# bharath5673/StrongSORT-YOLO

Hardware: AMD Instinct MI355X
Metric: tracked frames/sec (whole node), 1280x720@30det (higher is better)
Workload: dtype f32 association / f64 Kalman+LSAP (f16 detector convs, fp32 ReID network on own v_mfma_f32 kernels)

## Files before the change

strongsort_yolo_amd/csrc/ss_front.hip:

```cpp
#include <hip/hip_fp16.h>
#include "ss_common.h"

__device__ inline void ss_axis(int d, float scale, int n_src, int& i0, int& i1, float& frac)
{
    float t = (float)d + 0.5f;
    float s = t * scale;
    float f = s - 0.5f;
    int i = (int)floorf(f);
    float fr = f - (float)i;
    if (i < 0) { i = 0; fr = 0.0f; }
    if (i >= n_src - 1) { i = n_src - 1; fr = 0.0f; i1 = i; } else i1 = i + 1;
    i0 = i; frac = fr;
}

__device__ inline float ss_bilerp_u8(float p00, float p01, float p10, float p11, float fx, float fy)
{
    float a = fmaf(fx, p01 - p00, p00);
    float b = fmaf(fx, p11 - p10, p10);
    float v = fmaf(fy, b - a, a);
    float q = floorf(v + 0.5f);
    return fminf(fmaxf(q, 0.0f), 255.0f);
}

template <typename T> __device__ inline T ss_cvt(float v);
template <> __device__ inline float ss_cvt<float>(float v) { return v; }
template <> __device__ inline __half ss_cvt<__half>(float v) { return __float2half(v); }
template <typename T> struct ss_is_u8 { static constexpr bool value = false; };
template <> struct ss_is_u8<uint8_t> { static constexpr bool value = true; };

template <typename T, int HWC>
__global__ __launch_bounds__(256) void k_letterbox(const uint8_t* __restrict__ src, long long src_batch_stride,
                                                   int H, int W, int stride, T* __restrict__ dst, int out_h,
                                                   int out_w, int new_h, int new_w, int pad_top, int pad_left,
                                                   float padv)
{
    const int x = blockIdx.x * blockDim.x + threadIdx.x;
    const int y = blockIdx.y;
    if (x >= out_w) return;
    const size_t plane = (size_t)out_h * out_w;
    src += (size_t)blockIdx.z * src_batch_stride;
    dst += (size_t)blockIdx.z * 3 * plane;
    const size_t o = HWC ? ((size_t)y * out_w + x) * 3 : (size_t)y * out_w + x;
    const size_t cs = HWC ? 1 : plane;
    const int ry = y - pad_top, rx = x - pad_left;
    if (ry < 0 || ry >= new_h || rx < 0 || rx >= new_w) {
        T p = ss_cvt<T>(padv);
        dst[o] = p; dst[cs + o] = p; dst[2 * cs + o] = p;
        return;
    }
    const float sx = (float)W / (float)new_w, sy = (float)H / (float)new_h;
    int y0, y1, x0, x1; float fy, fx;
    ss_axis(ry, sy, H, y0, y1, fy);
    ss_axis(rx, sx, W, x0, x1, fx);
    const uint8_t* r0 = src + (size_t)y0 * stride;
    const uint8_t* r1 = src + (size_t)y1 * stride;
#pragma unroll
    for (int c = 0; c < 3; ++c) {
        const int sc = 2 - c;
        float p00 = r0[x0 * 3 + sc], p01 = r0[x1 * 3 + sc], p10 = r1[x0 * 3 + sc], p11 = r1[x1 * 3 + sc];
        dst[c * cs + o] = ss_cvt<T>(ss_bilerp_u8(p00, p01, p10, p11, fx, fy) / 255.0f);
    }
}

void ss_launch_letterbox(const uint8_t* src, int batch, long long src_batch_stride, int h, int w, int stride, void* dst,
                         int flags, int out_h, int out_w, int new_h, int new_w, int pad_top, int pad_left,
                         int pad_value, hipStream_t st)
{
    if (batch <= 0) return;
    dim3 grid((out_w + 255) / 256, out_h, batch), block(256);
    float padv = (float)pad_value / 255.0f;
#define SS_LB(T, L) hipLaunchKernelGGL((k_letterbox<T, L>), grid, block, 0, st, src, src_batch_stride, h, w, stride, \
                                       (T*)dst, out_h, out_w, new_h, new_w, pad_top, pad_left, padv)
    switch (flags & 3) {
    case 0: SS_LB(float, 0); break;
    case 1: SS_LB(__half, 0); break;
    case 2: SS_LB(float, 1); break;
    default: SS_LB(__half, 1); break;
    }
#undef SS_LB
}

template <typename T, int HWC>
__global__ __launch_bounds__(128) void k_crop(const uint8_t* __restrict__ src, long long src_batch_stride, int H, int W,
                                              int stride, const float* __restrict__ dets, int det_stride,
                                              long long dets_batch_stride, int n, const int* __restrict__ d_count,
                                              T* __restrict__ dst)
{
    const int out_w = 128, out_h = 256;
    const int img = blockIdx.z / n, d = blockIdx.z - img * n;
    const int cnt = d_count ? d_count[img] : n;
    if (d >= cnt) return;
    src += (size_t)img * src_batch_stride;
    const int x = threadIdx.x, y = blockIdx.y;
    const float* b = dets + (size_t)img * dets_batch_stride + (size_t)d * det_stride;
    int x1 = (int)b[0], y1 = (int)b[1], x2 = (int)b[2], y2 = (int)b[3];
    if (x1 < 0) x1 = 0; if (y1 < 0) y1 = 0;
    if (x2 > W - 1) x2 = W - 1; if (y2 > H - 1) y2 = H - 1;
    if (x1 > W - 1) x1 = W - 1; if (y1 > H - 1) y1 = H - 1;
    int cw = x2 - x1, ch = y2 - y1;
    if (cw < 1) cw = 1; if (ch < 1) ch = 1;
    const float sx = (float)cw / (float)out_w, sy = (float)ch / (float)out_h;
    int yy0, yy1, xx0, xx1; float fy, fx;
    ss_axis(y, sy, ch, yy0, yy1, fy);
    ss_axis(x, sx, cw, xx0, xx1, fx);
    const uint8_t* r0 = src + (size_t)(y1 + yy0) * stride;
    const uint8_t* r1 = src + (size_t)(y1 + yy1) * stride;
    const float mean[3] = { 0.485f, 0.456f, 0.406f }, sd[3] = { 0.229f, 0.224f, 0.225f };
    const size_t plane = (size_t)out_h * out_w;
    T* o = dst + (size_t)blockIdx.z * 3 * plane + (HWC ? ((size_t)y * out_w + x) * 3 : (size_t)y * out_w + x);
    const size_t cs = HWC ? 1 : plane;
#pragma unroll
    for (int c = 0; c < 3; ++c) {
        const int sc = 2 - c;
        float p00 = r0[(x1 + xx0) * 3 + sc], p01 = r0[(x1 + xx1) * 3 + sc];
        float p10 = r1[(x1 + xx0) * 3 + sc], p11 = r1[(x1 + xx1) * 3 + sc];
        float q = ss_bilerp_u8(p00, p01, p10, p11, fx, fy) / 255.0f;
        o[c * cs] = ss_cvt<T>((q - mean[c]) / sd[c]);
    }
}

#define CROP_LDS_BYTES 30720
#define CROP_RPT 4

template <typename T>
__global__ __launch_bounds__(256) void k_crop_hwc8(const uint8_t* __restrict__ src, long long src_batch_stride, int H, int W,
                                                   int stride, const float* __restrict__ dets, int det_stride,
                                                   long long dets_batch_stride, int n, const int* __restrict__ d_count,
                                                   T* __restrict__ dst, const int* __restrict__ d_off)
{
    extern __shared__ __attribute__((aligned(16))) unsigned char crop_smem[];
    T* lut = reinterpret_cast<T*>(crop_smem);
    uint32_t* Ls = reinterpret_cast<uint32_t*>(crop_smem + 768 * sizeof(T));
    const int out_w = 128, out_h = 256;
    const int img = blockIdx.z / n, d = blockIdx.z - img * n;
    const int cnt = d_count ? d_count[img] : n;
    if (d >= cnt) return;
    src += (size_t)img * src_batch_stride;
    const int tid = threadIdx.x, yb = blockIdx.y * (16 * CROP_RPT), xg = (tid & 15) * 8;
    const float* b = dets + (size_t)img * dets_batch_stride + (size_t)d * det_stride;
    int x1 = (int)b[0], y1 = (int)b[1], x2 = (int)b[2], y2 = (int)b[3];
    if (x1 < 0) x1 = 0; if (y1 < 0) y1 = 0;
    if (x2 > W - 1) x2 = W - 1; if (y2 > H - 1) y2 = H - 1;
    if (x1 > W - 1) x1 = W - 1; if (y1 > H - 1) y1 = H - 1;
    int cw = x2 - x1, ch = y2 - y1;
    if (cw < 1) cw = 1; if (ch < 1) ch = 1;
    const float sx = (float)cw / (float)out_w, sy = (float)ch / (float)out_h;
    const float mean[3] = { 0.485f, 0.456f, 0.406f }, sd[3] = { 0.229f, 0.224f, 0.225f };
    for (int i = tid; i < 768; i += 256) {
        const int c = i >> 8;
        const float q = (float)(i & 255) / 255.0f;
        if constexpr (ss_is_u8<T>::value) lut[i] = (uint8_t)(i & 255);
        else lut[i] = ss_cvt<T>((q - mean[c]) / sd[c]);
    }
    int ra0, ra1, rb0, rb1; float fa, fb;
    ss_axis(yb, sy, ch, ra0, ra1, fa);
    ss_axis(yb + 16 * CROP_RPT - 1, sy, ch, rb0, rb1, fb);
    const int nrows = rb1 - ra0 + 1;
    const size_t rowb = (size_t)x1 * 3;
    const int mis = (int)(rowb & 3), ndw = (mis + cw * 3 + 3) >> 2, pitch = ndw + 1;
    const bool aligned = (stride & 3) == 0 && ((uintptr_t)src & 3) == 0;
    bool fit_sub = aligned;
#pragma unroll
    for (int rr = 0; rr < CROP_RPT; ++rr) {
        int a0, a1, b0, b1; float f0, f1;
        ss_axis(yb + 16 * rr, sy, ch, a0, a1, f0);
        ss_axis(yb + 16 * rr + 15, sy, ch, b0, b1, f1);
        fit_sub = fit_sub && (size_t)(b1 - a0 + 1) * pitch * 4 <= CROP_LDS_BYTES;
    }
    const int mode = (aligned && (size_t)nrows * pitch * 4 <= CROP_LDS_BYTES) ? 2 : fit_sub ? 1 : 0;
    const bool staged = mode != 0;
    const size_t end = (size_t)H * stride;
    auto stage = [&](const int r_first, const int nr) {
        const int tot = nr * ndw;
        for (int i0 = tid; i0 < tot; i0 += 256 * 8) {
            uint32_t v[8];
            int la[8];
#pragma unroll
            for (int u = 0; u < 8; ++u) {
                const int i = i0 + 256 * u;
                v[u] = 0; la[u] = -1;
                if (i < tot) {
                    const int rr = i / ndw, dw = i - rr * ndw;
                    const size_t off = (size_t)(y1 + r_first + rr) * stride + (rowb - mis) + (size_t)dw * 4;
                    la[u] = rr * pitch + dw;
                    if (off + 4 <= end) v[u] = *reinterpret_cast<const uint32_t*>(src + off);
                    else { for (int k = 0; k < 4 && off + k < end; ++k) v[u] |= (uint32_t)src[off + k] << (8 * k); }
                }
            }
#pragma unroll
            for (int u = 0; u < 8; ++u) if (la[u] >= 0) Ls[la[u]] = v[u];
        }
    };
    if (mode == 2) stage(ra0, nrows);
    __syncthreads();
    const size_t slot = d_off ? (size_t)d_off[img] + d : (size_t)blockIdx.z;
    int hob0[8], hob1[8];
    float hfx[8];
#pragma unroll
    for (int p = 0; p < 8; ++p) {
        int xx0, xx1;
        ss_axis(xg + p, sx, cw, xx0, xx1, hfx[p]);
        hob0[p] = mis + 3 * xx0; hob1[p] = mis + 3 * xx1;
    }
#pragma unroll 1
    for (int rr = 0; rr < CROP_RPT; ++rr) {
    const int y = yb + rr * 16 + (tid >> 4);
    int yy0, yy1; float fy;
    ss_axis(y, sy, ch, yy0, yy1, fy);
    __attribute__((aligned(16))) T o[24];
    if (staged) {
        int row0 = ra0;
        if (mode == 1) {
            int a1, b0, b1; float f0, f1;
            ss_axis(yb + 16 * rr, sy, ch, row0, a1, f0);
            ss_axis(yb + 16 * rr + 15, sy, ch, b0, b1, f1);
            if (rr) __syncthreads();
            stage(row0, b1 - row0 + 1);
            __syncthreads();
        }
        const uint32_t* l0 = Ls + (yy0 - row0) * pitch;
        const uint32_t* l1 = Ls + (yy1 - row0) * pitch;
        auto px = [&](const uint32_t* row, int ob) -> uint32_t {
            const int dw = ob >> 2;
            const uint64_t two = ((uint64_t)row[dw + 1] << 32) | row[dw];
            return (uint32_t)(two >> (8 * (ob & 3)));
        };
#pragma unroll
        for (int p = 0; p < 8; ++p) {
            const float fx = hfx[p];
            const uint32_t v00 = px(l0, hob0[p]), v01 = px(l0, hob1[p]), v10 = px(l1, hob0[p]), v11 = px(l1, hob1[p]);
#pragma unroll
            for (int c = 0; c < 3; ++c) {
                const int sh = 8 * (2 - c);
                const float p00 = (float)((v00 >> sh) & 255u), p01 = (float)((v01 >> sh) & 255u), p10 = (float)((v10 >> sh) & 255u),
                            p11 = (float)((v11 >> sh) & 255u);
                o[p * 3 + c] = lut[c * 256 + (int)ss_bilerp_u8(p00, p01, p10, p11, fx, fy)];
            }
        }
    } else {
        const uint8_t* r0 = src + (size_t)(y1 + yy0) * stride + rowb;
        const uint8_t* r1 = src + (size_t)(y1 + yy1) * stride + rowb;
        T* od = dst + (slot * out_h * out_w + (size_t)y * out_w + xg) * 3;
#pragma unroll 1
        for (int p = 0; p < 8; ++p) {
            int xx0, xx1; float fx;
            ss_axis(xg + p, sx, cw, xx0, xx1, fx);
#pragma unroll
            for (int c = 0; c < 3; ++c) {
                const int sc = 2 - c;
                const float p00 = r0[xx0 * 3 + sc], p01 = r0[xx1 * 3 + sc], p10 = r1[xx0 * 3 + sc], p11 = r1[xx1 * 3 + sc];
                od[p * 3 + c] = lut[c * 256 + (int)ss_bilerp_u8(p00, p01, p10, p11, fx, fy)];
            }
        }
        continue;
    }
    if constexpr (ss_is_u8<T>::value) {
        uint2* out = reinterpret_cast<uint2*>(dst + (slot * out_h * out_w + (size_t)y * out_w + xg) * 3);
        const uint2* ov = reinterpret_cast<const uint2*>(o);
#pragma unroll
        for (int v = 0; v < 3; ++v) out[v] = ov[v];
    } else {
        constexpr int NV = 24 * sizeof(T) / 16;
        uint4* out = reinterpret_cast<uint4*>(dst + (slot * out_h * out_w + (size_t)y * out_w + xg) * 3);
        const uint4* ov = reinterpret_cast<const uint4*>(o);
#pragma unroll
        for (int v = 0; v < NV; ++v) out[v] = ov[v];
    }
    }
}

__global__ __launch_bounds__(1024) void k_crop_offsets(const int* __restrict__ counts, int batch, int n, int* __restrict__ off)
{
    __shared__ int wtot[16];
    const int tid = threadIdx.x, lane = tid & 63, wv = tid >> 6, per = (batch + 1023) / 1024, i0 = tid * per;
    int sum = 0;
    for (int i = i0; i < i0 + per && i < batch; ++i) sum += min(counts[i], n);
    int inc = sum;
#pragma unroll
    for (int o = 1; o < 64; o <<= 1) { const int t = __shfl_up(inc, o); if (lane >= o) inc += t; }
    if (lane == 63) wtot[wv] = inc;
    __syncthreads();
    int base = 0, total = 0;
#pragma unroll
    for (int i = 0; i < 16; ++i) { const int c = wtot[i]; if (i < wv) base += c; total += c; }
    int a = base + inc - sum;
    if (tid == 0) off[batch] = total;
    for (int i = i0; i < i0 + per && i < batch; ++i) { off[i] = a; a += min(counts[i], n); }
}

template <typename T>
__global__ __launch_bounds__(128) void k_unpack_feats(const T* __restrict__ emb, const int* __restrict__ off, const int* __restrict__ counts,
                                                     int n, float* __restrict__ feats, long long feats_img_stride)
{
    const int img = blockIdx.y, d = blockIdx.x;
    if (d >= min(counts[img], n)) return;
    const T* src = emb + ((size_t)off[img] + d) * 512;
    float* dst = feats + (size_t)img * feats_img_stride + (size_t)d * 512;
    for (int k = threadIdx.x; k < 512; k += 128) dst[k] = (float)src[k];
}

__global__ __launch_bounds__(256) void k_pack_results(const int* __restrict__ n_dets, const float* __restrict__ dets, int det_ld, int det_cap,
                                                      const int* __restrict__ n_out, const float* __restrict__ out, int out_ld, int out_cap,
                                                      float* __restrict__ dst)
{
    const int n = min(max(*n_dets, 0), det_cap), m = (n_out && out) ? min(max(*n_out, 0), out_cap) : 0;
    if (threadIdx.x == 0) { reinterpret_cast<int*>(dst)[0] = n; reinterpret_cast<int*>(dst)[1] = m; }
    float* d0 = dst + 2;
    for (int i = threadIdx.x; i < n * det_ld; i += 256) d0[i] = dets[i];
    float* d1 = dst + 2 + (size_t)det_cap * det_ld;
    for (int i = threadIdx.x; i < m * out_ld; i += 256) d1[i] = out[i];
}

void ss_launch_pack_results(const int* n_dets, const float* dets, int det_ld, int det_cap, const int* n_out, const float* out, int out_ld,
                            int out_cap, float* dst, hipStream_t st)
{ hipLaunchKernelGGL(k_pack_results, dim3(1), dim3(256), 0, st, n_dets, dets, det_ld, det_cap, n_out, out, out_ld, out_cap, dst); }

void ss_launch_crop_offsets(const int* counts, int batch, int n, int* off, hipStream_t st)
{ hipLaunchKernelGGL(k_crop_offsets, dim3(1), dim3(1024), 0, st, counts, batch, n, off); }

void ss_launch_unpack_feats(const void* emb, int half, const int* off, const int* counts, int batch, int n, float* feats,
                            long long feats_img_stride, hipStream_t st)
{
    if (batch <= 0 || n <= 0) return;
    if (half) hipLaunchKernelGGL(k_unpack_feats<__half>, dim3(n, batch), dim3(128), 0, st, (const __half*)emb, off, counts, n, feats, feats_img_stride);
    else hipLaunchKernelGGL(k_unpack_feats<float>, dim3(n, batch), dim3(128), 0, st, (const float*)emb, off, counts, n, feats, feats_img_stride);
}

void ss_launch_crop(const uint8_t* frame, int batch, long long frame_batch_stride, int h, int w, int stride,
                    const float* dets, int det_stride, long long dets_batch_stride, int n, const int* d_count,
                    void* out, int flags, hipStream_t st, const int* d_off)
{
    if (n <= 0 || batch <= 0) return;
    if (flags & 2) {
        dim3 grid(1, 16 / CROP_RPT, n * batch), block(256);
        if (flags & 4) { hipLaunchKernelGGL(k_crop_hwc8<uint8_t>, grid, block, 768 + CROP_LDS_BYTES + 8, st, frame, frame_batch_stride, h, w, stride, dets, det_stride, dets_batch_stride, n, d_count, (uint8_t*)out, d_off); return; }
        if (flags & 1) hipLaunchKernelGGL(k_crop_hwc8<__half>, grid, block, 768 * sizeof(__half) + CROP_LDS_BYTES + 8, st, frame, frame_batch_stride, h, w, stride, dets, det_stride, dets_batch_stride, n, d_count, (__half*)out, d_off);
        else           hipLaunchKernelGGL(k_crop_hwc8<float>, grid, block, 768 * sizeof(float) + CROP_LDS_BYTES + 8, st, frame, frame_batch_stride, h, w, stride, dets, det_stride, dets_batch_stride, n, d_count, (float*)out, d_off);
        return;
    }
    dim3 grid(1, 256, n * batch), block(128);
#define SS_CR(T, L) hipLaunchKernelGGL((k_crop<T, L>), grid, block, 0, st, frame, frame_batch_stride, h, w, stride, dets, \
                                       det_stride, dets_batch_stride, n, d_count, (T*)out)
    if (flags & 1) SS_CR(__half, 0); else SS_CR(float, 0);
#undef SS_CR
}

#define NMS_MAX_ANCHORS 32768
#define NMS_MAX_CAND 8192
#define NMS_WORDS (NMS_MAX_CAND / 64)

struct NmsWs {
    unsigned long long* keys;
    int* cand_cls;
    float* box;
    float* area;
    unsigned long long* mask;
    int* counters;
};

size_t ss_nms_workspace_bytes()
{
    return (size_t)NMS_MAX_ANCHORS * 8 + (size_t)NMS_MAX_ANCHORS * 4 + (size_t)NMS_MAX_CAND * 16 +
           (size_t)NMS_MAX_CAND * 4 + (size_t)NMS_MAX_CAND * NMS_WORDS * 8 + 64;
}

__host__ __device__ inline NmsWs carve_nms(void* ws)
{
    NmsWs w; char* p = (char*)ws;
    w.keys = (unsigned long long*)p; p += (size_t)NMS_MAX_ANCHORS * 8;
    w.mask = (unsigned long long*)p; p += (size_t)NMS_MAX_CAND * NMS_WORDS * 8;
    w.box = (float*)p; p += (size_t)NMS_MAX_CAND * 16;
    w.area = (float*)p; p += (size_t)NMS_MAX_CAND * 4;
    w.cand_cls = (int*)p; p += (size_t)NMS_MAX_ANCHORS * 4;
    w.counters = (int*)p;
    return w;
}

struct NmsBatch {
    const float* pred; long long pred_stride;
    char* ws; long long ws_stride;
};
__device__ inline NmsWs nms_unit(const NmsBatch& nb, int img) { return carve_nms(nb.ws + (size_t)img * nb.ws_stride); }

__global__ __launch_bounds__(512) void k_nms_filter(NmsBatch nb, int N, int nc, float conf, unsigned long long cm0,
                                                    unsigned long long cm1)
{
    const float* __restrict__ pred = nb.pred + (size_t)blockIdx.y * nb.pred_stride;
    const NmsWs w = nms_unit(nb, blockIdx.y);
    __shared__ float sbest[8][64];
    __shared__ int scls[8][64];
    const int g = threadIdx.x >> 6, l = threadIdx.x & 63;
    const int a = blockIdx.x * 64 + l;
    float best = -INFINITY; int bc = 0x7fffffff;
    if (a < N)
        for (int k0 = g; k0 < nc; k0 += 80) {
            float s[10];
#pragma unroll
            for (int j = 0; j < 10; ++j) s[j] = pred[(size_t)(4 + min(k0 + 8 * j, nc - 1)) * N + a];
#pragma unroll
            for (int j = 0; j < 10; ++j) {
                const int k = k0 + 8 * j;
                if (k < nc && s[j] > best) { best = s[j]; bc = k; }
            }
        }
    sbest[g][l] = best; scls[g][l] = bc;
    __syncthreads();
    if (g != 0 || a >= N) return;
#pragma unroll
    for (int q = 1; q < 8; ++q) {
        float s = sbest[q][l]; int c = scls[q][l];
        if (s > best || (s == best && c < bc)) { best = s; bc = c; }
    }
    const bool allowed = bc < 64 ? (cm0 >> bc) & 1ull : bc < 128 ? (cm1 >> (bc - 64)) & 1ull : true;
    if (best > conf && allowed) {
        int slot = atomicAdd(&w.counters[0], 1);
        w.keys[slot] = ((unsigned long long)(~__float_as_uint(best)) << 32) | (unsigned)a;
        w.cand_cls[a] = bc;
    }
}

__global__ __launch_bounds__(1024) void k_nms_sort(NmsBatch nb, int N, int agnostic, float max_wh)
{
    const float* __restrict__ pred = nb.pred + (size_t)blockIdx.x * nb.pred_stride;
    const NmsWs w = nms_unit(nb, blockIdx.x);
    extern __shared__ __attribute__((aligned(16))) char smem[];
    unsigned long long* k = (unsigned long long*)smem;
    int n = w.counters[0];
    __syncthreads();
    if (n > NMS_MAX_CAND) {
        if (threadIdx.x == 0) { w.counters[1] = SS_ERR_CAPACITY; w.counters[0] = 0; }
        n = 0;
    }
    int np = 1; while (np < n) np <<= 1;
    for (int i = threadIdx.x; i < np; i += 1024) k[i] = i < n ? w.keys[i] : ~0ull;
    __syncthreads();
    for (int size = 2; size <= np; size <<= 1)
        for (int strd = size >> 1; strd > 0; strd >>= 1) {
            for (int i = threadIdx.x; i < np / 2; i += 1024) {
                int lo = 2 * i - (i & (strd - 1)), hi = lo + strd;
                bool up = (lo & size) == 0;
                unsigned long long a = k[lo], b = k[hi];
                if ((a > b) == up) { k[lo] = b; k[hi] = a; }
            }
            __syncthreads();
        }
    for (int i = threadIdx.x; i < n; i += 1024) {
        unsigned long long key = k[i];
        w.keys[i] = key;
        const int a = (int)(key & 0xffffffffu);
        float cx = pred[a], cy = pred[(size_t)N + a], bw = pred[(size_t)2 * N + a], bh = pred[(size_t)3 * N + a];
        float hw = bw / 2.0f, hh = bh / 2.0f;
        float off = agnostic ? 0.0f : (float)w.cand_cls[a] * max_wh;
        float x1 = (cx - hw) + off, y1 = (cy - hh) + off, x2 = (cx + hw) + off, y2 = (cy + hh) + off;
        w.box[i * 4 + 0] = x1; w.box[i * 4 + 1] = y1; w.box[i * 4 + 2] = x2; w.box[i * 4 + 3] = y2;
        w.area[i] = (x2 - x1) * (y2 - y1);
    }
}

#define NMS_MASK_WG 256
__global__ __launch_bounds__(64) void k_nms_mask(NmsBatch nb, float iou_thres)
{
    const NmsWs w = nms_unit(nb, blockIdx.y);
    __shared__ float sb[64 * 4];
    __shared__ float sa[64];
    const int n = min(w.counters[0], NMS_MAX_CAND);
    const int nblk = (n + 63) / 64;
    const int npair = nblk * (nblk + 1) / 2;
    const int t = threadIdx.x;
    for (int pr = blockIdx.x; pr < npair; pr += gridDim.x) {
        int ib = 0, rem = pr;
        while (rem >= nblk - ib) { rem -= nblk - ib; ++ib; }
        const int jb = ib + rem;
        const int j = jb * 64 + t;
        __syncthreads();
        if (j < n) { sb[t * 4] = w.box[j * 4]; sb[t * 4 + 1] = w.box[j * 4 + 1]; sb[t * 4 + 2] = w.box[j * 4 + 2]; sb[t * 4 + 3] = w.box[j * 4 + 3]; sa[t] = w.area[j]; }
        __syncthreads();
        const int i = ib * 64 + t;
        if (i >= n) continue;
        const float x1 = w.box[i * 4], y1 = w.box[i * 4 + 1], x2 = w.box[i * 4 + 2], y2 = w.box[i * 4 + 3], ai = w.area[i];
        unsigned long long bits = 0;
        const int jn = min(64, n - jb * 64);
        for (int q = 0; q < jn; ++q) {
            if (jb * 64 + q <= i) continue;
            float xx1 = fmaxf(x1, sb[q * 4]), yy1 = fmaxf(y1, sb[q * 4 + 1]);
            float xx2 = fminf(x2, sb[q * 4 + 2]), yy2 = fminf(y2, sb[q * 4 + 3]);
            float iw = fmaxf(0.0f, xx2 - xx1), ih = fmaxf(0.0f, yy2 - yy1);
            float inter = iw * ih;
            float iou = inter / (ai + sa[q] - inter);
            if (iou > iou_thres) bits |= 1ull << q;
        }
        w.mask[(size_t)i * NMS_WORDS + jb] = bits;
    }
}

__global__ __launch_bounds__(64) void k_nms_scan(NmsBatch nb, int N, int nc, int n_extra, int max_det, float gain,
                                                 float pad_x, float pad_y, float w0, float h0,
                                                 const float* __restrict__ geom, float* __restrict__ rows,
                                                 int row_stride, long long rows_batch_stride, int* __restrict__ keep,
                                                 long long keep_batch_stride, int* __restrict__ count)
{
    const int img = blockIdx.x;
    const float* __restrict__ pred = nb.pred + (size_t)img * nb.pred_stride;
    const NmsWs w = nms_unit(nb, img);
    rows += (size_t)img * rows_batch_stride; keep += (size_t)img * keep_batch_stride; count += img;
    if (geom) { const float* g = geom + img * 5; gain = g[0]; pad_x = g[1]; pad_y = g[2]; w0 = g[3]; h0 = g[4]; }
    __shared__ int kept_sorted[1024];
    const int n = min(w.counters[0], NMS_MAX_CAND);
    const int l = threadIdx.x;
    const int nw = (n + 63) / 64;
    unsigned long long rem0 = 0, rem1 = 0;
    int kept = 0;
    const int cap = min(max_det, 1024);
    for (int ib = 0; ib < nw && kept < cap; ++ib) {
        unsigned long long rw = __shfl((ib < 64) ? rem0 : rem1, ib & 63);
        const int i0 = ib * 64;
        const int cnt = min(64, n - i0);
        unsigned long long diag = (l < cnt) ? w.mask[(size_t)(i0 + l) * NMS_WORDS + ib] : 0ull;
        unsigned long long keptbits = 0;
        for (int q = 0; q < cnt && kept < cap; ++q) {
            if (!((rw >> q) & 1ull)) {
                keptbits |= 1ull << q;
                if (l == 0) kept_sorted[kept] = i0 + q;
                ++kept;
                rw |= __shfl(diag, q);
            }
        }
        unsigned long long kb = keptbits;
        while (kb) {
            int q[4];
#pragma unroll
            for (int u = 0; u < 4; ++u) { q[u] = kb ? __builtin_ctzll(kb) : -1; if (kb) kb &= kb - 1; }
            unsigned long long a0[4], a1[4];
#pragma unroll
            for (int u = 0; u < 4; ++u) {
                a0[u] = a1[u] = 0ull;
                if (q[u] >= 0) {
                    const unsigned long long* mr = w.mask + (size_t)(i0 + q[u]) * NMS_WORDS;
                    if (l > ib && l < nw) a0[u] = mr[l];
                    if (l + 64 > ib && l + 64 < nw) a1[u] = mr[l + 64];
                }
            }
            rem0 |= (a0[0] | a0[1]) | (a0[2] | a0[3]);
            rem1 |= (a1[0] | a1[1]) | (a1[2] | a1[3]);
        }
    }
    __syncthreads();
    if (l == 0) { *count = kept; w.counters[0] = 0; }
    for (int kk = l; kk < kept; kk += 64) {
        const int i = kept_sorted[kk];
        const unsigned long long key = w.keys[i];
        const int a = (int)(key & 0xffffffffu);
        const float score = __uint_as_float(~(unsigned)(key >> 32));
        float cx = pred[a], cy = pred[(size_t)N + a], bw = pred[(size_t)2 * N + a], bh = pred[(size_t)3 * N + a];
        float hw = bw / 2.0f, hh = bh / 2.0f;
        float x1 = ((cx - hw) - pad_x) / gain, y1 = ((cy - hh) - pad_y) / gain;
        float x2 = ((cx + hw) - pad_x) / gain, y2 = ((cy + hh) - pad_y) / gain;
        float* r = rows + (size_t)kk * row_stride;
        r[0] = fminf(fmaxf(x1, 0.0f), w0); r[1] = fminf(fmaxf(y1, 0.0f), h0);
        r[2] = fminf(fmaxf(x2, 0.0f), w0); r[3] = fminf(fmaxf(y2, 0.0f), h0);
        r[4] = score; r[5] = (float)w.cand_cls[a];
        for (int e = 0; e < n_extra; ++e) r[6 + e] = pred[(size_t)(4 + nc + e) * N + a];
        keep[kk] = a;
    }
}

__global__ __launch_bounds__(1024) void k_nms_rest(NmsBatch nb, int N, int nc, int n_extra, int agnostic, float max_wh, float iou_thres,
                                                   int max_det, float gain, float pad_x, float pad_y, float w0, float h0,
                                                   const float* __restrict__ geom, float* __restrict__ rows, int row_stride,
                                                   long long rows_batch_stride, int* __restrict__ keep, long long keep_batch_stride,
                                                   int* __restrict__ count)
{
    const int img = blockIdx.x;
    const float* __restrict__ pred = nb.pred + (size_t)img * nb.pred_stride;
    const NmsWs w = nms_unit(nb, img);
    rows += (size_t)img * rows_batch_stride; keep += (size_t)img * keep_batch_stride; count += img;
    if (geom) { const float* g = geom + img * 5; gain = g[0]; pad_x = g[1]; pad_y = g[2]; w0 = g[3]; h0 = g[4]; }
    extern __shared__ __attribute__((aligned(16))) char smem[];
    unsigned long long* k = (unsigned long long*)smem;
    float* sbw = (float*)(smem + (size_t)NMS_MAX_CAND * 8);
    float* saw = sbw + 16 * 64 * 4;
    int* kept_sorted = (int*)(saw + 16 * 64);
    __shared__ int s_kept;
    const int tid = threadIdx.x, l = tid & 63, wv = tid >> 6;
    int n = w.counters[0];
    __syncthreads();
    if (n > NMS_MAX_CAND) {
        if (tid == 0) { w.counters[1] = SS_ERR_CAPACITY; w.counters[0] = 0; }
        n = 0;
    }
    if (n <= 64) {
        if (wv == 0) {
            unsigned long long key = l < n ? w.keys[l] : ~0ull;
            auto shfl64 = [](unsigned long long v, int src) {
                const unsigned lo = (unsigned)__shfl((int)(unsigned)v, src), hi = (unsigned)__shfl((int)(unsigned)(v >> 32), src);
                return ((unsigned long long)hi << 32) | lo;
            };
#pragma unroll
            for (int size = 2; size <= 64; size <<= 1)
#pragma unroll
                for (int strd = size >> 1; strd > 0; strd >>= 1) {
                    const unsigned long long other = shfl64(key, l ^ strd);
                    const bool lower = (l & strd) == 0, up = (l & size) == 0;
                    const bool take_min = lower == up;
                    key = take_min ? (key < other ? key : other) : (key > other ? key : other);
                }
            float x1 = 0.f, y1 = 0.f, x2 = 0.f, y2 = 0.f, ai = 0.f;
            if (l < n) {
                w.keys[l] = key;
                const int a = (int)(key & 0xffffffffu);
                float cx = pred[a], cy = pred[(size_t)N + a], bw = pred[(size_t)2 * N + a], bh = pred[(size_t)3 * N + a];
                float hw = bw / 2.0f, hh = bh / 2.0f;
                float off = agnostic ? 0.0f : (float)w.cand_cls[a] * max_wh;
                x1 = (cx - hw) + off; y1 = (cy - hh) + off; x2 = (cx + hw) + off; y2 = (cy + hh) + off;
                ai = (x2 - x1) * (y2 - y1);
                sbw[l * 4] = x1; sbw[l * 4 + 1] = y1; sbw[l * 4 + 2] = x2; sbw[l * 4 + 3] = y2; saw[l] = ai;
            }
            SS_WAVE_SYNC();
            unsigned long long bits = 0;
            if (l < n) {
                for (int q = 0; q < n; ++q) {
                    if (q <= l) continue;
                    float xx1 = fmaxf(x1, sbw[q * 4]), yy1 = fmaxf(y1, sbw[q * 4 + 1]);
                    float xx2 = fminf(x2, sbw[q * 4 + 2]), yy2 = fminf(y2, sbw[q * 4 + 3]);
                    float iw = fmaxf(0.0f, xx2 - xx1), ih = fmaxf(0.0f, yy2 - yy1);
                    float inter = iw * ih;
                    float iou = inter / (ai + saw[q] - inter);
                    if (iou > iou_thres) bits |= 1ull << q;
                }
            }
            unsigned long long rw = 0;
            int kept = 0;
            const int cap = min(max_det, 1024);
            for (int q = 0; q < n && kept < cap; ++q) {
                if (!((rw >> q) & 1ull)) {
                    if (l == 0) kept_sorted[kept] = q;
                    ++kept;
                    rw |= shfl64(bits, q);
// ... 160 lines not shown
```

strongsort_yolo_amd/csrc/ss_ops.hip:

```cpp
#include <hip/hip_fp16.h>
#include <hip/hip_runtime.h>
#include <stdint.h>
#include <stdlib.h>
#include <string>
#include "../../include/strongsort_hip.h"

struct NvEntry { void* stream; const int* n; int batch; };
static thread_local NvEntry g_nv[8] = {};
static inline const int* nv_for(void* stream, long long batch)
{
    for (const NvEntry& e : g_nv) if (e.n && e.stream == stream && e.batch == batch) return e.n;
    return nullptr;
}
static inline int nv_batch(void* stream)
{
    for (const NvEntry& e : g_nv) if (e.n && e.stream == stream) return e.batch;
    return 0;
}

static int g_opt_pw_epilogue = 1, g_opt_pw_splitk = 1, g_opt_osnet_chains = 1;

typedef _Float16 h8 __attribute__((ext_vector_type(8)));
typedef _Float16 h4 __attribute__((ext_vector_type(4)));
typedef float f4 __attribute__((ext_vector_type(4)));

__device__ inline float act_apply(float v, int act)
{
    if (act == 1) return v > 0.f ? v : 0.f;
    if (act == 2) return v * __builtin_amdgcn_rcpf(1.0f + __expf(-v));
    if (act == 3) return __builtin_amdgcn_rcpf(1.0f + __expf(-v));
    return v;
}

__global__ __launch_bounds__(256) void k_bias_act8(__half* __restrict__ x, const __half* __restrict__ bias,
                                                  const __half* __restrict__ res, size_t n_vec, int C8, int act)
{
    for (size_t i = blockIdx.x * (size_t)blockDim.x + threadIdx.x; i < n_vec; i += (size_t)gridDim.x * blockDim.x) {
        h8 v = reinterpret_cast<h8*>(x)[i];
        h8 b = reinterpret_cast<const h8*>(bias)[i % C8];
        h8 r;
        if (res) r = reinterpret_cast<const h8*>(res)[i];
#pragma unroll
        for (int k = 0; k < 8; ++k) {
            float f = (float)v[k] + (float)b[k];
            if (res) f += (float)r[k];
            v[k] = (_Float16)act_apply(f, act);
        }
        reinterpret_cast<h8*>(x)[i] = v;
    }
}

__global__ __launch_bounds__(256) void k_bias_act1(__half* __restrict__ x, const __half* __restrict__ bias,
                                                  const __half* __restrict__ res, size_t n, int C, int act)
{
    for (size_t i = blockIdx.x * (size_t)blockDim.x + threadIdx.x; i < n; i += (size_t)gridDim.x * blockDim.x) {
        float f = __half2float(x[i]) + __half2float(bias[i % C]);
        if (res) f += __half2float(res[i]);
        x[i] = __float2half(act_apply(f, act));
    }
}

__device__ __forceinline__ float ss_mix_lo(unsigned a, unsigned b, float c)
{ float d; asm("v_fma_mix_f32 %0, %1, %2, %3 op_sel:[0,0,0] op_sel_hi:[1,1,0]" : "=v"(d) : "v"(a), "v"(b), "v"(c)); return d; }
__device__ __forceinline__ float ss_mix_hi(unsigned a, unsigned b, float c)
{ float d; asm("v_fma_mix_f32 %0, %1, %2, %3 op_sel:[1,1,0] op_sel_hi:[1,1,0]" : "=v"(d) : "v"(a), "v"(b), "v"(c)); return d; }
__device__ __forceinline__ void ss_dw_tap8(const h8& v, const h8& w, float (&acc)[8])
{
    const uint4 vu = __builtin_bit_cast(uint4, v), wu = __builtin_bit_cast(uint4, w);
    acc[0] = ss_mix_lo(vu.x, wu.x, acc[0]); acc[1] = ss_mix_hi(vu.x, wu.x, acc[1]);
    acc[2] = ss_mix_lo(vu.y, wu.y, acc[2]); acc[3] = ss_mix_hi(vu.y, wu.y, acc[3]);
    acc[4] = ss_mix_lo(vu.z, wu.z, acc[4]); acc[5] = ss_mix_hi(vu.z, wu.z, acc[5]);
    acc[6] = ss_mix_lo(vu.w, wu.w, acc[6]); acc[7] = ss_mix_hi(vu.w, wu.w, acc[7]);
}

__global__ __launch_bounds__(256) void k_dw3x3(const __half* __restrict__ x, const __half* __restrict__ w9,
                                              const __half* __restrict__ bias, __half* __restrict__ y, int N, int H,
                                              int W, int C8, int act)
{
    const size_t total = (size_t)N * H * W * C8;
    for (size_t i = blockIdx.x * (size_t)blockDim.x + threadIdx.x; i < total; i += (size_t)gridDim.x * blockDim.x) {
        const int c8 = (int)(i % C8);
        const size_t p = i / C8;
        const int w = (int)(p % W), h = (int)((p / W) % H);
        const size_t nb = (p / ((size_t)W * H)) * H;
        float acc[8];
        {
            h8 b = reinterpret_cast<const h8*>(bias)[c8];
#pragma unroll
            for (int k = 0; k < 8; ++k) acc[k] = (float)b[k];
        }
#pragma unroll
        for (int dy = -1; dy <= 1; ++dy) {
            const int hh = h + dy;
            if (hh < 0 || hh >= H) continue;
#pragma unroll
            for (int dx = -1; dx <= 1; ++dx) {
                const int ww = w + dx;
                if (ww < 0 || ww >= W) continue;
                h8 v = reinterpret_cast<const h8*>(x)[((nb + hh) * W + ww) * C8 + c8];
                h8 k9 = reinterpret_cast<const h8*>(w9)[((dy + 1) * 3 + dx + 1) * C8 + c8];
                ss_dw_tap8(v, k9, acc);
            }
        }
        h8 o;
#pragma unroll
        for (int k = 0; k < 8; ++k) o[k] = (_Float16)act_apply(acc[k], act);
        reinterpret_cast<h8*>(y)[i] = o;
    }
}

__global__ __launch_bounds__(256) void k_bias_act_place(const __half* __restrict__ x, const __half* __restrict__ bias,
                                                       const __half* __restrict__ res, size_t n_vec, int C8, int act,
                                                       int res_after, __half* __restrict__ out, int out_ld8,
                                                       __half* __restrict__ out2, int c0_8, int cn_8)
{
    for (size_t i = blockIdx.x * (size_t)blockDim.x + threadIdx.x; i < n_vec; i += (size_t)gridDim.x * blockDim.x) {
        const size_t pix = i / C8;
        const int c8 = (int)(i - pix * C8);
        h8 v = reinterpret_cast<const h8*>(x)[i];
        const h8 b = reinterpret_cast<const h8*>(bias)[c8];
        h8 r;
        if (res) r = reinterpret_cast<const h8*>(res)[i];
#pragma unroll
        for (int k = 0; k < 8; ++k) {
            float f = (float)v[k] + (float)b[k];
            if (res && !res_after) f += (float)r[k];
            f = act_apply(f, act);
            if (res && res_after) f = (float)(_Float16)f + (float)r[k];
            v[k] = (_Float16)f;
        }
        reinterpret_cast<h8*>(out)[pix * out_ld8 + c8] = v;
        if (out2 && c8 >= c0_8 && c8 < c0_8 + cn_8) reinterpret_cast<h8*>(out2)[pix * cn_8 + (c8 - c0_8)] = v;
    }
}

struct V8Levels {
    const __half* box[3]; const __half* cls[3];
    const __half* box_bias[3]; const __half* cls_bias[3];
    int H[3], W[3], stride[3];
    const __half* ext[3];
    int n_ext, ext_ld, ext_mode;
    int cls_ld;
};

__global__ __launch_bounds__(128) void k_v8_decode(V8Levels L, int B, int nc, int A, float* __restrict__ pred)
{
    const int a = blockIdx.x * blockDim.x + threadIdx.x, b = blockIdx.y;
    if (a >= A) return;
    int l = 0, a0 = 0;
    while (l < 2 && a >= a0 + L.H[l] * L.W[l]) { a0 += L.H[l] * L.W[l]; ++l; }
    const int p = a - a0, hw = L.H[l] * L.W[l];
    const int py = p / L.W[l], px = p - py * L.W[l];
    const h8* bx = reinterpret_cast<const h8*>(L.box[l] + ((size_t)b * hw + p) * 64);
    const h8* bb = reinterpret_cast<const h8*>(L.box_bias[l]);
    float d[4];
#pragma unroll
    for (int s = 0; s < 4; ++s) {
        float v[16], m = -INFINITY;
#pragma unroll
        for (int h = 0; h < 2; ++h) {
            const h8 t = bx[s * 2 + h], tb = bb[s * 2 + h];
#pragma unroll
            for (int k = 0; k < 8; ++k) { v[h * 8 + k] = (float)t[k] + (float)tb[k]; m = fmaxf(m, v[h * 8 + k]); }
        }
        float se = 0.f, sw = 0.f;
#pragma unroll
        for (int k = 0; k < 16; ++k) { const float e = __expf(v[k] - m); se += e; sw += e * (float)k; }
        d[s] = sw / se;
    }
    const float ax = (float)px + 0.5f, ay = (float)py + 0.5f, st = (float)L.stride[l];
    const float x1 = ax - d[0], y1 = ay - d[1], x2 = ax + d[2], y2 = ay + d[3];
    float* o = pred + (size_t)b * (4 + nc + L.n_ext) * A + a;
    o[0] = (x1 + x2) * 0.5f * st; o[(size_t)A] = (y1 + y2) * 0.5f * st;
    o[(size_t)2 * A] = (x2 - x1) * st; o[(size_t)3 * A] = (y2 - y1) * st;
    if (L.n_ext) {
        const __half* e = L.ext[l] + ((size_t)b * hw + p) * L.ext_ld;
        float* oe = o + (size_t)(4 + nc) * A;
        for (int k = 0, j = 0; k < L.n_ext; ++k, j = j == 2 ? 0 : j + 1) {
            const float v = __half2float(e[k]);
            oe[(size_t)k * A] = L.ext_mode == 0 ? v : j == 0 ? (v * 2.0f + (float)px) * st : j == 1 ? (v * 2.0f + (float)py) * st : 1.0f / (1.0f + __expf(-v));
        }
    }
    const __half* cl = L.cls[l] + ((size_t)b * hw + p) * L.cls_ld;
    const __half* cb = L.cls_bias[l];
    if (nc % 8 == 0) {
        for (int k8 = 0; k8 < nc / 8; ++k8) {
            const h8 t = reinterpret_cast<const h8*>(cl)[k8], tb = reinterpret_cast<const h8*>(cb)[k8];
#pragma unroll
            for (int k = 0; k < 8; ++k) o[(size_t)(4 + k8 * 8 + k) * A] = 1.0f / (1.0f + __expf(-((float)t[k] + (float)tb[k])));
        }
        return;
    }
    for (int k = 0; k < nc; ++k) {
        const float z = __half2float(cl[k]) + __half2float(cb[k]);
        o[(size_t)(4 + k) * A] = 1.0f / (1.0f + __expf(-z));
    }
}

struct ConvGeom { int H, W, Cin, OH, OW, stride; };

struct PwArgs {
    const __half* x; const __half* w; const __half* bias; const __half* res;
    int M, K, N, act, res_after;
    __half* out; int out_ld; __half* out2; int c0, cn;
    ConvGeom g;
    const int* n_img; int img_px;
};

template <int BN, int PT, bool VEC_EPI>
constexpr int pw_lds_halfs() { return BN * 72 + (VEC_EPI ? 4 * PT * 16 * (BN + 8) : 0); }

template <int BN, int PT, bool CONV3, bool VEC_EPI>
__device__ __forceinline__ void pw_body(const PwArgs& A, const int bx, const int by, _Float16* __restrict__ pw_lds)
{
    const __half* __restrict__ x = A.x; const __half* __restrict__ w = A.w; const __half* __restrict__ bias = A.bias;
    const __half* __restrict__ res = A.res; __half* __restrict__ out = A.out; __half* __restrict__ out2 = A.out2;
    const int K = A.K, N = A.N, act = A.act, res_after = A.res_after, out_ld = A.out_ld, c0 = A.c0, cn = A.cn;
    int M = A.M;
    if (A.n_img) { const long long mv = (long long)(*A.n_img) * A.img_px; if (mv < M) M = (int)mv; }
    const ConvGeom g = A.g;
    constexpr int MT = BN / 16, KC = 64, PITCH = KC + 8, BM = 64 * PT;
    if ((long long)bx * BM >= M) return;
    _Float16* __restrict__ Ws = pw_lds;
    const int tid = threadIdx.x, lane = tid & 63, wave = tid >> 6, q = lane >> 4, n = lane & 15;
    const int n0 = by * BN;
    const size_t px0 = (size_t)bx * BM + wave * (16 * PT);
    f4 acc[MT][PT];
#pragma unroll
    for (int mt = 0; mt < MT; ++mt)
#pragma unroll
        for (int pt = 0; pt < PT; ++pt) acc[mt][pt] = f4{ 0.f, 0.f, 0.f, 0.f };
    const h8 z8 = { 0, 0, 0, 0, 0, 0, 0, 0 };
    size_t ibase[PT];
    int iy0[PT], ix0[PT];
    if (CONV3) {
#pragma unroll
        for (int pt = 0; pt < PT; ++pt) {
            const size_t px = px0 + pt * 16 + n;
            const int ohw = g.OH * g.OW;
            const int bimg = (int)(px / ohw), rem = (int)(px - (size_t)bimg * ohw), oy = rem / g.OW, ox = rem - oy * g.OW;
            ibase[pt] = (size_t)bimg * g.H * g.W;
            iy0[pt] = oy * g.stride - 1; ix0[pt] = ox * g.stride - 1;
        }
    }

    constexpr int WV = (BN * (KC / 8) + 255) / 256;
    auto load_w = [&](int kc, h8 (&wr)[WV]) {
#pragma unroll
        for (int j = 0; j < WV; ++j) {
            const int i = tid + j * 256, r = i / (KC / 8), c8 = i - r * (KC / 8);
            const int oc = n0 + r, k = kc + c8 * 8;
            wr[j] = (i < BN * (KC / 8) && oc < N && k < K) ? *reinterpret_cast<const h8*>(w + (size_t)oc * K + k) : z8;
        }
    };
    auto load_b = [&](int kc, h8 (&b)[KC / 32][PT]) {
#pragma unroll
        for (int ks = 0; ks < KC / 32; ++ks)
#pragma unroll
            for (int pt = 0; pt < PT; ++pt) {
                const size_t px = px0 + pt * 16 + n;
                const int k = kc + ks * 32 + 8 * q;
                if (!CONV3) {
                    b[ks][pt] = (px < (size_t)M && k < K) ? *reinterpret_cast<const h8*>(x + px * K + k) : z8;
                } else {
                    const int tap = k / g.Cin, c = k - tap * g.Cin, dy = tap / 3, dx = tap - dy * 3;
                    const int iy = iy0[pt] + dy, ix = ix0[pt] + dx;
                    const bool ok = px < (size_t)M && k < K && iy >= 0 && iy < g.H && ix >= 0 && ix < g.W;
                    b[ks][pt] = ok ? *reinterpret_cast<const h8*>(x + (ibase[pt] + (size_t)iy * g.W + ix) * g.Cin + c) : z8;
                }
            }
    };
    h8 wr[WV], wn[WV], b[KC / 32][PT], bn[KC / 32][PT];
    load_w(0, wr);
    load_b(0, b);
    for (int kc = 0; kc < K; kc += KC) {
        __syncthreads();
#pragma unroll
        for (int j = 0; j < WV; ++j) {
            const int i = tid + j * 256, r = i / (KC / 8), c8 = i - r * (KC / 8);
            if (i < BN * (KC / 8)) *reinterpret_cast<h8*>(Ws + r * PITCH + c8 * 8) = wr[j];
        }
        if (kc + KC < K) { load_w(kc + KC, wn); load_b(kc + KC, bn); }
        __syncthreads();
#pragma unroll
        for (int ks = 0; ks < KC / 32; ++ks) {
            if (kc + ks * 32 >= K) break;
#pragma unroll
            for (int mt = 0; mt < MT; ++mt) {
                const h8 a = *reinterpret_cast<const h8*>(Ws + (mt * 16 + n) * PITCH + ks * 32 + 8 * q);
                const h4 a0 = { a[0], a[1], a[2], a[3] }, a1 = { a[4], a[5], a[6], a[7] };
#pragma unroll
                for (int pt = 0; pt < PT; ++pt) {
                    const h8 bv = b[ks][pt];
                    if (CONV3) {
                        acc[mt][pt] = __builtin_amdgcn_mfma_f32_16x16x32_f16(a, bv, acc[mt][pt], 0, 0, 0);
                    } else {
                        const h4 b0 = { bv[0], bv[1], bv[2], bv[3] }, b1 = { bv[4], bv[5], bv[6], bv[7] };
                        acc[mt][pt] = __builtin_amdgcn_mfma_f32_16x16x16f16(a0, b0, acc[mt][pt], 0, 0, 0);
                        acc[mt][pt] = __builtin_amdgcn_mfma_f32_16x16x16f16(a1, b1, acc[mt][pt], 0, 0, 0);
                    }
                }
            }
        }
        if (kc + KC < K) {
#pragma unroll
            for (int j = 0; j < WV; ++j) wr[j] = wn[j];
#pragma unroll
            for (int ks = 0; ks < KC / 32; ++ks)
#pragma unroll
                for (int pt = 0; pt < PT; ++pt) b[ks][pt] = bn[ks][pt];
        }
    }

    if (VEC_EPI) {
        constexpr int EP = BN + 8;
        _Float16* tile = pw_lds + BN * PITCH + wave * (PT * 16 * EP);
#pragma unroll
        for (int pt = 0; pt < PT; ++pt)
#pragma unroll
            for (int mt = 0; mt < MT; ++mt) {
                const h4 o = { (_Float16)acc[mt][pt][0], (_Float16)acc[mt][pt][1], (_Float16)acc[mt][pt][2], (_Float16)acc[mt][pt][3] };
                *reinterpret_cast<h4*>(tile + (pt * 16 + n) * EP + mt * 16 + 4 * q) = o;
            }
        __builtin_amdgcn_wave_barrier();
        constexpr int CG = BN / 8;
#pragma unroll
        for (int it = 0; it < (PT * 16 * CG + 63) / 64; ++it) {
            const int i = it * 64 + lane, row = i / CG, cg = i - row * CG;
            const size_t px = px0 + row;
            const int oc = n0 + cg * 8;
            if (i >= PT * 16 * CG || px >= (size_t)M || oc >= N) continue;
            const h8 v = *reinterpret_cast<const h8*>(tile + row * EP + cg * 8);
            const h8 bb = *reinterpret_cast<const h8*>(bias + oc);
            h8 r = z8;
            if (res) r = *reinterpret_cast<const h8*>(res + px * N + oc);
            h8 o;
#pragma unroll
            for (int j = 0; j < 8; ++j) {
                float f = (float)v[j] + (float)bb[j];
                if (res && !res_after) f += (float)r[j];
                f = act_apply(f, act);
                if (res && res_after) f = (float)(_Float16)f + (float)r[j];
                o[j] = (_Float16)f;
            }
            *reinterpret_cast<h8*>(out + px * out_ld + oc) = o;
            if (out2 && oc >= c0 && oc < c0 + cn) *reinterpret_cast<h8*>(out2 + px * cn + (oc - c0)) = o;
        }
        return;
    }
#pragma unroll
    for (int pt = 0; pt < PT; ++pt) {
        const size_t px = px0 + pt * 16 + n;
        if (px >= (size_t)M) continue;
#pragma unroll
        for (int mt = 0; mt < MT; ++mt) {
            const int oc0 = n0 + mt * 16 + 4 * q;
            if (oc0 >= N) continue;
            const h4 bb = *reinterpret_cast<const h4*>(bias + oc0);
            h4 r = { 0, 0, 0, 0 };
            if (res) r = *reinterpret_cast<const h4*>(res + px * N + oc0);
            h4 o;
#pragma unroll
            for (int j = 0; j < 4; ++j) {
                float f = (float)(_Float16)acc[mt][pt][j] + (float)bb[j];
                if (res && !res_after) f += (float)r[j];
                f = act_apply(f, act);
                if (res && res_after) f = (float)(_Float16)f + (float)r[j];
                o[j] = (_Float16)f;
            }
            *reinterpret_cast<h4*>(out + px * out_ld + oc0) = o;
            if (out2 && oc0 >= c0 && oc0 < c0 + cn) *reinterpret_cast<h4*>(out2 + px * cn + (oc0 - c0)) = o;
        }
    }
}

#ifndef SS_TAIL_BUMP
#define SS_TAIL_BUMP 1
#endif
#ifndef SS_PW_BUMP
#define SS_PW_BUMP 1
#endif
template <int BN, int PT, bool CONV3> constexpr int pw_waves() { return !SS_PW_BUMP ? 1 : BN * PT <= 32 ? 8 : (BN == 32 && PT == 2 && CONV3) ? 5 : BN * PT <= 80 ? 6 : BN * PT <= 128 ? 4 : BN * PT <= 160 ? 3 : 2; }
template <int BN, int PT, bool CONV3, bool VEC_EPI>
__global__ __launch_bounds__(256) __attribute__((amdgpu_waves_per_eu(pw_waves<BN, PT, CONV3>()))) void k_pw(PwArgs A)
{
    __shared__ __attribute__((aligned(16))) _Float16 pw_lds[pw_lds_halfs<BN, PT, VEC_EPI>()];
    pw_body<BN, PT, CONV3, VEC_EPI>(A, blockIdx.x, blockIdx.y, pw_lds);
}

template <int BN, bool CONV3>
__device__ __forceinline__ void pw_splitk_body(const PwArgs& A, const int bx, const int by)
{
    const __half* __restrict__ x = A.x; const __half* __restrict__ w = A.w; const __half* __restrict__ bias = A.bias;
    const __half* __restrict__ res = A.res; __half* __restrict__ out = A.out; __half* __restrict__ out2 = A.out2;
    const int K = A.K, N = A.N, act = A.act, res_after = A.res_after, out_ld = A.out_ld, c0 = A.c0, cn = A.cn;
    int M = A.M;
    if (A.n_img) { const long long mv = (long long)(*A.n_img) * A.img_px; if (mv < M) M = (int)mv; }
    const ConvGeom g = A.g;
    constexpr int MT = BN / 16, KC = 64, RP = 17;
    __shared__ float Red[4 * BN * RP];
    const int tid = threadIdx.x, lane = tid & 63, wave = tid >> 6, q = lane >> 4, n = lane & 15;
    const int n0 = by * BN;
    const size_t px = (size_t)bx * 16 + n;
    const h8 z8 = { 0, 0, 0, 0, 0, 0, 0, 0 };
    size_t ibase = 0;
    int iy0 = 0, ix0 = 0;
    if (CONV3) {
        const int ohw = g.OH * g.OW;
        const int bimg = (int)(px / ohw), rem = (int)(px - (size_t)bimg * ohw), oy = rem / g.OW, ox = rem - oy * g.OW;
        ibase = (size_t)bimg * g.H * g.W;
        iy0 = oy * g.stride - 1; ix0 = ox * g.stride - 1;
    }
    auto load_a = [&](int kc, h8 (&a)[MT][2]) {
#pragma unroll
        for (int mt = 0; mt < MT; ++mt)
#pragma unroll
            for (int ks = 0; ks < 2; ++ks) {
                const int oc = n0 + mt * 16 + n, k = kc + ks * 32 + 8 * q;
                a[mt][ks] = (oc < N && k < K) ? *reinterpret_cast<const h8*>(w + (size_t)oc * K + k) : z8;
            }
    };
    auto load_b = [&](int kc, h8 (&b)[2]) {
#pragma unroll
        for (int ks = 0; ks < 2; ++ks) {
            const int k = kc + ks * 32 + 8 * q;
            if (!CONV3) {
                b[ks] = (px < (size_t)M && k < K) ? *reinterpret_cast<const h8*>(x + px * K + k) : z8;
            } else {
                const int tap = k / g.Cin, c = k - tap * g.Cin, dy = tap / 3, dx = tap - dy * 3;
                const int iy = iy0 + dy, ix = ix0 + dx;
                const bool ok = px < (size_t)M && k < K && iy >= 0 && iy < g.H && ix >= 0 && ix < g.W;
                b[ks] = ok ? *reinterpret_cast<const h8*>(x + (ibase + (size_t)iy * g.W + ix) * g.Cin + c) : z8;
            }
        }
    };
    f4 acc[MT];
#pragma unroll
    for (int mt = 0; mt < MT; ++mt) acc[mt] = f4{ 0.f, 0.f, 0.f, 0.f };
    h8 a[MT][2], b[2], an[MT][2], bn[2];
    int kc = wave * KC;
    if (kc < K) { load_a(kc, a); load_b(kc, b); }
    for (; kc < K; kc += 4 * KC) {
        const bool more = kc + 4 * KC < K;
        if (more) { load_a(kc + 4 * KC, an); load_b(kc + 4 * KC, bn); }
#pragma unroll
        for (int ks = 0; ks < 2; ++ks) {
            if (kc + ks * 32 >= K) break;
#pragma unroll
            for (int mt = 0; mt < MT; ++mt) acc[mt] = __builtin_amdgcn_mfma_f32_16x16x32_f16(a[mt][ks], b[ks], acc[mt], 0, 0, 0);
        }
        if (more) {
#pragma unroll
            for (int mt = 0; mt < MT; ++mt) { a[mt][0] = an[mt][0]; a[mt][1] = an[mt][1]; }
            b[0] = bn[0]; b[1] = bn[1];
        }
    }
#pragma unroll
    for (int mt = 0; mt < MT; ++mt)
#pragma unroll
        for (int j = 0; j < 4; ++j) Red[(wave * BN + mt * 16 + 4 * q + j) * RP + n] = acc[mt][j];
    __syncthreads();
    constexpr int CG = BN / 8;
    if (tid < 16 * CG) {
        const int row = tid / CG, cg = tid - row * CG;
        const size_t p = (size_t)bx * 16 + row;
        const int oc = n0 + cg * 8;
        if (p < (size_t)M && oc < N) {
            const h8 bb = *reinterpret_cast<const h8*>(bias + oc);
            h8 r = z8;
            if (res) r = *reinterpret_cast<const h8*>(res + p * N + oc);
            h8 o;
#pragma unroll
            for (int j = 0; j < 8; ++j) {
                const int ch = cg * 8 + j;
                const float sum = ((Red[(0 * BN + ch) * RP + row] + Red[(1 * BN + ch) * RP + row]) + Red[(2 * BN + ch) * RP + row]) +
                                  Red[(3 * BN + ch) * RP + row];
                float f = (float)(_Float16)sum + (float)bb[j];
                if (res && !res_after) f += (float)r[j];
                f = act_apply(f, act);
                if (res && res_after) f = (float)(_Float16)f + (float)r[j];
                o[j] = (_Float16)f;
            }
            *reinterpret_cast<h8*>(out + p * out_ld + oc) = o;
            if (out2 && oc >= c0 && oc < c0 + cn) *reinterpret_cast<h8*>(out2 + p * cn + (oc - c0)) = o;
        }
    }
}

template <int BN, bool CONV3>
__global__ __launch_bounds__(256) void k_pw_splitk(PwArgs A) { pw_splitk_body<BN, CONV3>(A, blockIdx.x, blockIdx.y); }

#define PW_GROUP_MAX 12
struct PwGroup { PwArgs p[PW_GROUP_MAX]; int start[PW_GROUP_MAX + 1]; int form[PW_GROUP_MAX]; int n; };

#ifndef SS_GRP_WAVES
#define SS_GRP_WAVES 6
#endif
template <int BN, bool CONV3, bool SPLITK>
__global__ __launch_bounds__(256)
__attribute__((amdgpu_waves_per_eu(SPLITK || !SS_GRP_WAVES ? 1 : SS_GRP_WAVES)))
void k_pw_group(PwGroup G)
{
    __shared__ __attribute__((aligned(16))) _Float16 pw_lds[pw_lds_halfs<BN, 1, true>()];
    int bx = blockIdx.x, p = 0;
    for (int i = 1; i < G.n; ++i) if (bx >= G.start[i]) p = i;
    bx -= G.start[p];
    const int form = G.form[p];
    if constexpr (SPLITK) { if (form == 1) { pw_splitk_body<BN, CONV3>(G.p[p], bx, 0); return; } }
    if (BN == 80 && G.p[p].N <= 64) pw_body<64, 1, CONV3, true>(G.p[p], bx, 0, pw_lds);
    else pw_body<BN, 1, CONV3, true>(G.p[p], bx, 0, pw_lds);
}

struct BnArgs {
    const __half* x; const __half* w1; const __half* b1; const __half* w2; const __half* b2;
    __half* out; int out_ld; __half* out2;
    int B, H, W, add, TW, TH, tiles_x, tiles_y;
};

template <int CI, int CO, int PT>
__device__ __forceinline__ void bn_conv(const _Float16* __restrict__ In, const int (&pbase)[PT], const int* __restrict__ tapoff,
                                        const __half* __restrict__ w, _Float16* __restrict__ Ws, f4 (&acc)[CO / 16][PT], const int tid)
{
    constexpr int C = CI;
    constexpr int MT = CO / 16, WP = 72, K = 9 * CI, WV = (CO * 8 + 255) / 256;
    const int lane = tid & 63, q = lane >> 4, n = lane & 15;
    const h8 z8 = { 0, 0, 0, 0, 0, 0, 0, 0 };
    auto load_w = [&](int k0, h8 (&wr)[WV]) {
#pragma unroll
        for (int j = 0; j < WV; ++j) {
            const int i = tid + j * 256, r = i >> 3, c8 = i & 7, kk = k0 + c8 * 8;
            wr[j] = (i < CO * 8 && kk < K) ? *reinterpret_cast<const h8*>(w + (size_t)r * K + kk) : z8;
        }
    };
    h8 wr[WV], wn[WV];
    load_w(0, wr);
    int buf = 0;
    for (int k0 = 0; k0 < K; k0 += 64, buf ^= 1) {
        _Float16* wb = Ws + buf * (CO * WP);
#pragma unroll
        for (int j = 0; j < WV; ++j) {
            const int i = tid + j * 256, r = i >> 3, c8 = i & 7;
            if (i < CO * 8) *reinterpret_cast<h8*>(wb + r * WP + c8 * 8) = wr[j];
        }
        if (k0 + 64 < K) load_w(k0 + 64, wn);
        __syncthreads();
        h8 b[2][PT], a[2][MT];
#pragma unroll
        for (int ks = 0; ks < 2; ++ks) {
            const int kk = k0 + ks * 32 + 8 * q, tap = kk / C, c = kk % C;
            const bool kv = kk < K;
            const int boff = kv ? tapoff[tap] + c : 0;
#pragma unroll
            for (int pt = 0; pt < PT; ++pt) {
                b[ks][pt] = *reinterpret_cast<const h8*>(In + pbase[pt] + boff);
                if (!kv) b[ks][pt] = z8;
            }
#pragma unroll
            for (int mt = 0; mt < MT; ++mt) a[ks][mt] = *reinterpret_cast<const h8*>(wb + (mt * 16 + n) * WP + ks * 32 + 8 * q);
        }
#pragma unroll
        for (int ks = 0; ks < 2; ++ks) {
            if (k0 + ks * 32 >= K) break;
#pragma unroll
            for (int mt = 0; mt < MT; ++mt)
#pragma unroll
                for (int pt = 0; pt < PT; ++pt)
                    acc[mt][pt] = __builtin_amdgcn_mfma_f32_16x16x32_f16(a[ks][mt], b[ks][pt], acc[mt][pt], 0, 0, 0);
        }
        if (k0 + 64 < K) {
#pragma unroll
            for (int j = 0; j < WV; ++j) wr[j] = wn[j];
        }
    }
}

template <int C, int PT1, int PT2>
__global__ __launch_bounds__(256) __attribute__((amdgpu_waves_per_eu(!SS_TAIL_BUMP ? 1 : C == 16 ? 6 : 1))) void k_bneck(BnArgs A)
{
    extern __shared__ __attribute__((aligned(16))) char bn_smem[];
    constexpr int MT = C / 16, P = C + 8, WP = 72;
    const int tid = threadIdx.x, lane = tid & 63, wave = tid >> 6, q = lane >> 4, n = lane & 15;
    const int TW = A.TW, TH = A.TH, XW = TW + 4, XH = TH + 4, RW = TW + 2, RH = TH + 2;
    _Float16* Xs = reinterpret_cast<_Float16*>(bn_smem);
    _Float16* Ts = Xs + XH * XW * P;
    _Float16* Ws = Ts + ((RH * RW * P + 7) & ~7);
    int* tap1 = reinterpret_cast<int*>(Ws + 2 * C * WP);
    int* tap2 = tap1 + 16;
    const int tpi = A.tiles_x * A.tiles_y;
    const int img = blockIdx.x / tpi, trm = blockIdx.x - img * tpi, tyi = trm / A.tiles_x, txi = trm - tyi * A.tiles_x;
    const int oy0 = tyi * TH, ox0 = txi * TW, H = A.H, W = A.W;
    const h8 z8 = { 0, 0, 0, 0, 0, 0, 0, 0 };
    if (tid < 9) { const int ky = tid / 3, kx = tid - ky * 3; tap1[tid] = (ky * XW + kx) * P; tap2[tid] = (ky * RW + kx) * P; }
    const __half* xi = A.x + (size_t)img * H * W * C;
    constexpr int VPC = C / 8;
    const int rowv = XW * VPC;
    for (int r = wave; r < XH; r += 4) {
        const int iy = oy0 - 2 + r;
        const bool rok = iy >= 0 && iy < H;
        const __half* src = xi + (size_t)(rok ? iy : 0) * W * C;
        _Float16* dst = Xs + r * XW * P;
        for (int i0 = lane; i0 < rowv; i0 += 512) {
            h8 tmp[8];
#pragma unroll
            for (int u = 0; u < 8; ++u) {
                const int i = i0 + 64 * u, c = i / VPC, v = i % VPC, ix = ox0 - 2 + c;
                const bool ok = rok && i < rowv && ix >= 0 && ix < W;
                tmp[u] = ok ? *reinterpret_cast<const h8*>(src + (size_t)ix * C + v * 8) : z8;
            }
#pragma unroll
            for (int u = 0; u < 8; ++u) {
                const int i = i0 + 64 * u, c = i / VPC, v = i % VPC;
                if (i < rowv) *reinterpret_cast<h8*>(dst + c * P + v * 8) = tmp[u];
            }
        }
    }
    {
        int pb[PT1], tpix[PT1];
        bool inimg[PT1];
#pragma unroll
        for (int pt = 0; pt < PT1; ++pt) {
            const int p = (wave * PT1 + pt) * 16 + n;
            int ry = p / RW, rx = p - ry * RW;
            const bool ok = p < RH * RW;
            if (!ok) { ry = 0; rx = 0; }
            const int iy = oy0 - 1 + ry, ix = ox0 - 1 + rx;
            inimg[pt] = ok && iy >= 0 && iy < H && ix >= 0 && ix < W;
            tpix[pt] = ok ? p : -1;
            pb[pt] = (ry * XW + rx) * P;
        }
        f4 acc[MT][PT1];
#pragma unroll
        for (int mt = 0; mt < MT; ++mt)
#pragma unroll
            for (int pt = 0; pt < PT1; ++pt) acc[mt][pt] = f4{ 0.f, 0.f, 0.f, 0.f };
        bn_conv<C, C, PT1>(Xs, pb, tap1, A.w1, Ws, acc, tid);
#pragma unroll
        for (int mt = 0; mt < MT; ++mt) {
            const h4 bb = *reinterpret_cast<const h4*>(A.b1 + mt * 16 + 4 * q);
#pragma unroll
            for (int pt = 0; pt < PT1; ++pt) {
                if (tpix[pt] < 0) continue;
                h4 o;
#pragma unroll
                for (int j = 0; j < 4; ++j) {
                    float f = act_apply((float)(_Float16)acc[mt][pt][j] + (float)bb[j], 2);
                    asm volatile("" : "+v"(f));
                    o[j] = inimg[pt] ? (_Float16)f : (_Float16)0.f;
                }
                *reinterpret_cast<h4*>(Ts + tpix[pt] * P + mt * 16 + 4 * q) = o;
            }
        }
    }
    __syncthreads();
    {
        int pb[PT2], opix[PT2], xoff[PT2];
#pragma unroll
        for (int pt = 0; pt < PT2; ++pt) {
            const int p = (wave * PT2 + pt) * 16 + n;
            int ty = p / TW, tx = p - ty * TW;
            const bool ok = p < TH * TW && oy0 + ty < H && ox0 + tx < W;
            if (!ok) { ty = 0; tx = 0; }
            pb[pt] = (ty * RW + tx) * P;
            xoff[pt] = ((ty + 2) * XW + tx + 2) * P;
            opix[pt] = ok ? (img * H + oy0 + ty) * W + ox0 + tx : -1;
        }
        f4 acc[MT][PT2];
#pragma unroll
        for (int mt = 0; mt < MT; ++mt)
#pragma unroll
            for (int pt = 0; pt < PT2; ++pt) acc[mt][pt] = f4{ 0.f, 0.f, 0.f, 0.f };
        bn_conv<C, C, PT2>(Ts, pb, tap2, A.w2, Ws, acc, tid);
#pragma unroll
        for (int mt = 0; mt < MT; ++mt) {
            const h4 bb = *reinterpret_cast<const h4*>(A.b2 + mt * 16 + 4 * q);
#pragma unroll
            for (int pt = 0; pt < PT2; ++pt) {
                if (opix[pt] < 0) continue;
                const h4 xr = *reinterpret_cast<const h4*>(Xs + xoff[pt] + mt * 16 + 4 * q);
                h4 o;
#pragma unroll
                for (int j = 0; j < 4; ++j) {
                    float f = act_apply((float)(_Float16)acc[mt][pt][j] + (float)bb[j], 2);
                    asm volatile("" : "+v"(f));
                    if (A.add) f = (float)(_Float16)f + (float)xr[j];
                    o[j] = (_Float16)f;
                }
                *reinterpret_cast<h4*>(A.out + (size_t)opix[pt] * A.out_ld + mt * 16 + 4 * q) = o;
                if (A.out2) *reinterpret_cast<h4*>(A.out2 + (size_t)opix[pt] * C + mt * 16 + 4 * q) = o;
            }
        }
    }
}

struct HeadArgs {
    const __half* x;
    const __half* w1[2]; const __half* b1[2]; const __half* w2[2]; const __half* b2[2]; const __half* w3[2]; const __half* b3[2];
    __half* out[2]; int nout[2];
    int B, H, W, TW, TH, tiles_x, tiles_y;
};

template <int CI, int CM, int PT1, int PT2>
__device__ __forceinline__ void head_body(const HeadArgs& A, const int br, char* smem)
{
    constexpr int MT = CM / 16, PX = CI + 8, PM = CM + 8, WP = 72, KB3 = (CM + 31) / 32;
    const int tid = threadIdx.x, lane = tid & 63, wave = tid >> 6, q = lane >> 4, n = lane & 15;
    const int TW = A.TW, TH = A.TH, XW = TW + 4, XH = TH + 4, RW = TW + 2, RH = TH + 2;
    _Float16* Xs = reinterpret_cast<_Float16*>(smem);
    _Float16* Ts = Xs + ((XH * XW * PX + 7) & ~7);
    _Float16* Ws = Ts + ((RH * RW * PM + 7) & ~7);
    int* tap1 = reinterpret_cast<int*>(Ws + 2 * 80 * WP);
    int* tap2 = tap1 + 16;
    _Float16* Us = Xs;
    const int tpi = A.tiles_x * A.tiles_y;
    const int img = blockIdx.x / tpi, trm = blockIdx.x - img * tpi, tyi = trm / A.tiles_x, txi = trm - tyi * A.tiles_x;
    const int oy0 = tyi * TH, ox0 = txi * TW, H = A.H, W = A.W;
    const h8 z8 = { 0, 0, 0, 0, 0, 0, 0, 0 };
    if (tid < 9) { const int ky = tid / 3, kx = tid - ky * 3; tap1[tid] = (ky * XW + kx) * PX; tap2[tid] = (ky * RW + kx) * PM; }
    const __half* xi = A.x + (size_t)img * H * W * CI;
    constexpr int VPC = CI / 8;
    const int rowv = XW * VPC;
    for (int r = wave; r < XH; r += 4) {
        const int iy = oy0 - 2 + r;
        const bool rok = iy >= 0 && iy < H;
        const __half* src = xi + (size_t)(rok ? iy : 0) * W * CI;
        _Float16* dst = Xs + r * XW * PX;
        for (int i0 = lane; i0 < rowv; i0 += 512) {
            h8 tmp[8];
#pragma unroll
            for (int u = 0; u < 8; ++u) {
                const int i = i0 + 64 * u, c = i / VPC, v = i % VPC, ix = ox0 - 2 + c;
                const bool ok = rok && i < rowv && ix >= 0 && ix < W;
                tmp[u] = ok ? *reinterpret_cast<const h8*>(src + (size_t)ix * CI + v * 8) : z8;
            }
#pragma unroll
            for (int u = 0; u < 8; ++u) {
                const int i = i0 + 64 * u, c = i / VPC, v = i % VPC;
                if (i < rowv) *reinterpret_cast<h8*>(dst + c * PX + v * 8) = tmp[u];
            }
        }
    }
    {
        int pb[PT1], tpix[PT1];
        bool inimg[PT1];
#pragma unroll
        for (int pt = 0; pt < PT1; ++pt) {
            const int p = (wave * PT1 + pt) * 16 + n;
            int ry = p / RW, rx = p - ry * RW;
            const bool ok = p < RH * RW;
            if (!ok) { ry = 0; rx = 0; }
            const int iy = oy0 - 1 + ry, ix = ox0 - 1 + rx;
            inimg[pt] = ok && iy >= 0 && iy < H && ix >= 0 && ix < W;
            tpix[pt] = ok ? p : -1;
            pb[pt] = (ry * XW + rx) * PX;
        }
        f4 acc[MT][PT1];
#pragma unroll
        for (int mt = 0; mt < MT; ++mt)
#pragma unroll
            for (int pt = 0; pt < PT1; ++pt) acc[mt][pt] = f4{ 0.f, 0.f, 0.f, 0.f };
        bn_conv<CI, CM, PT1>(Xs, pb, tap1, A.w1[br], Ws, acc, tid);
#pragma unroll
        for (int mt = 0; mt < MT; ++mt) {
            const h4 bb = *reinterpret_cast<const h4*>(A.b1[br] + mt * 16 + 4 * q);
#pragma unroll
            for (int pt = 0; pt < PT1; ++pt) {
                if (tpix[pt] < 0) continue;
                h4 o;
#pragma unroll
                for (int j = 0; j < 4; ++j) {
                    float f = act_apply((float)(_Float16)acc[mt][pt][j] + (float)bb[j], 2);
                    asm volatile("" : "+v"(f));
                    o[j] = inimg[pt] ? (_Float16)f : (_Float16)0.f;
                }
                *reinterpret_cast<h4*>(Ts + tpix[pt] * PM + mt * 16 + 4 * q) = o;
            }
        }
    }
    __syncthreads();
    int opix[PT2];
    {
        int pb[PT2];
#pragma unroll
        for (int pt = 0; pt < PT2; ++pt) {
            const int p = (wave * PT2 + pt) * 16 + n;
            int ty = p / TW, tx = p - ty * TW;
            const bool ok = p < TH * TW && oy0 + ty < H && ox0 + tx < W;
            if (!ok) { ty = 0; tx = 0; }
            pb[pt] = (ty * RW + tx) * PM;
            opix[pt] = ok ? (img * H + oy0 + ty) * W + ox0 + tx : -1;
        }
        f4 acc[MT][PT2];
#pragma unroll
        for (int mt = 0; mt < MT; ++mt)
#pragma unroll
            for (int pt = 0; pt < PT2; ++pt) acc[mt][pt] = f4{ 0.f, 0.f, 0.f, 0.f };
        bn_conv<CM, CM, PT2>(Ts, pb, tap2, A.w2[br], Ws, acc, tid);
        _Float16* ut = Us + wave * (PT2 * 16 * PM);
#pragma unroll
        for (int mt = 0; mt < MT; ++mt) {
            const h4 bb = *reinterpret_cast<const h4*>(A.b2[br] + mt * 16 + 4 * q);
#pragma unroll
            for (int pt = 0; pt < PT2; ++pt) {
                h4 o;
#pragma unroll
                for (int j = 0; j < 4; ++j) {
                    float f = act_apply((float)(_Float16)acc[mt][pt][j] + (float)bb[j], 2);
                    asm volatile("" : "+v"(f));
                    o[j] = (_Float16)f;
                }
                *reinterpret_cast<h4*>(ut + (pt * 16 + n) * PM + mt * 16 + 4 * q) = o;
            }
        }
    }
    __syncthreads();
    const int nout = A.nout[br];
    {
        const __half* w3 = A.w3[br];
        for (int i = tid; i < CM * (CM / 8); i += 256) {
            const int r = i / (CM / 8), c8 = i - r * (CM / 8);
            *reinterpret_cast<h8*>(Ws + r * PM + c8 * 8) = r < nout ? *reinterpret_cast<const h8*>(w3 + (size_t)r * CM + c8 * 8) : z8;
        }
    }
    __syncthreads();
    {
        const _Float16* ut = Us + wave * (PT2 * 16 * PM);
        f4 acc[MT][PT2];
#pragma unroll
        for (int mt = 0; mt < MT; ++mt)
#pragma unroll
            for (int pt = 0; pt < PT2; ++pt) acc[mt][pt] = f4{ 0.f, 0.f, 0.f, 0.f };
#pragma unroll
        for (int kb = 0; kb < KB3; ++kb) {
            const int k = kb * 32 + 8 * q;
            const bool kv = k < CM;
            h8 b[PT2];
#pragma unroll
            for (int pt = 0; pt < PT2; ++pt) b[pt] = kv ? *reinterpret_cast<const h8*>(ut + (pt * 16 + n) * PM + k) : z8;
#pragma unroll
            for (int mt = 0; mt < MT; ++mt) {
                const h8 a = kv ? *reinterpret_cast<const h8*>(Ws + (mt * 16 + n) * PM + k) : z8;
                const h4 a0 = { a[0], a[1], a[2], a[3] }, a1 = { a[4], a[5], a[6], a[7] };
#pragma unroll
                for (int pt = 0; pt < PT2; ++pt) {
                    const h4 b0 = { b[pt][0], b[pt][1], b[pt][2], b[pt][3] }, b1 = { b[pt][4], b[pt][5], b[pt][6], b[pt][7] };
                    acc[mt][pt] = __builtin_amdgcn_mfma_f32_16x16x16f16(a0, b0, acc[mt][pt], 0, 0, 0);
                    acc[mt][pt] = __builtin_amdgcn_mfma_f32_16x16x16f16(a1, b1, acc[mt][pt], 0, 0, 0);
                }
            }
        }
        __half* out = A.out[br];
#pragma unroll
        for (int mt = 0; mt < MT; ++mt) {
            const int oc0 = mt * 16 + 4 * q;
            if (oc0 >= nout) continue;
            const h4 bb = *reinterpret_cast<const h4*>(A.b3[br] + oc0);
#pragma unroll
            for (int pt = 0; pt < PT2; ++pt) {
                if (opix[pt] < 0) continue;
                h4 o;
#pragma unroll
                for (int j = 0; j < 4; ++j) o[j] = (_Float16)((float)(_Float16)acc[mt][pt][j] + (float)bb[j]);
                *reinterpret_cast<h4*>(out + (size_t)opix[pt] * nout + oc0) = o;
            }
        }
    }
}

template <int CI, int PT1, int PT2>
__global__ __launch_bounds__(256) void k_head(HeadArgs A)
{
    extern __shared__ __attribute__((aligned(16))) char hd_smem[];
    if (blockIdx.y == 0) head_body<CI, 64, PT1, PT2>(A, 0, hd_smem);
    else head_body<CI, 80, PT1, PT2>(A, 1, hd_smem);
}

#define STEM_W 128
#define STEM_M 16
#define STEM_PITCH 416
#define STEM_IN_ROWS 23
#define STEM_CR 9
#define STEM_CW 65
#define STEM_CP 18
typedef _Float16 h4a4 __attribute__((ext_vector_type(4), aligned(4)));
typedef _Float16 h8a4 __attribute__((ext_vector_type(8), aligned(4)));

__global__ __launch_bounds__(256) void k_osnet_stem(const __half* __restrict__ x, const __half* __restrict__ wp ,
                                                   const __half* __restrict__ bias, __half* __restrict__ y, int H, int tiles,
                                                   const int* __restrict__ nvalid, const __half* __restrict__ w1c,
                                                   const __half* __restrict__ b1c, __half* __restrict__ y1)
{
    if (nvalid && (int)(blockIdx.x / tiles) >= *nvalid) return;
    __shared__ __attribute__((aligned(16))) _Float16 In[STEM_IN_ROWS * STEM_PITCH];
    __shared__ __attribute__((aligned(16))) _Float16 Cv[STEM_CR * STEM_CW * STEM_CP];
    const int tid = threadIdx.x, lane = tid & 63, r = tid >> 6, q = lane >> 4, n = lane & 15;
    const int img = blockIdx.x / tiles, j0 = (blockIdx.x - img * tiles) * 4;
    const int OHc = H / 2, OHp = OHc / 2;
    const int in_r0 = 4 * j0 - 5, cv_r0 = 2 * j0 - 1;
    const h8 z8 = { 0, 0, 0, 0, 0, 0, 0, 0 };

    const __half* xi = x + (size_t)img * H * STEM_W * 3;
    constexpr int CH = STEM_PITCH / 8;
    {
        constexpr int NIT = (STEM_IN_ROWS * CH + 255) / 256;
        h8 v[NIT];
#pragma unroll
        for (int it = 0; it < NIT; ++it) {
            const int i = min(tid + 256 * it, STEM_IN_ROWS * CH - 1);
            const int rr = i / CH, ch = i - rr * CH;
            const int gr = min(max(in_r0 + rr, 0), H - 1), cc = min(max(ch - STEM_M / 8, 0), STEM_W * 3 / 8 - 1);
            v[it] = *reinterpret_cast<const h8*>(xi + (size_t)gr * STEM_W * 3 + cc * 8);
        }
#pragma unroll
        for (int it = 0; it < NIT; ++it) {
            const int i = tid + 256 * it;
            if (i < STEM_IN_ROWS * CH) {
                const int rr = i / CH, ch = i - rr * CH, gr = in_r0 + rr;
                const bool ok = ch >= STEM_M / 8 && ch < STEM_M / 8 + STEM_W * 3 / 8 && gr >= 0 && gr < H;
                *reinterpret_cast<h8*>(In + rr * STEM_PITCH + ch * 8) = ok ? v[it] : z8;
            }
        }
    }
    if (tid < STEM_CR * 2) *reinterpret_cast<h8a4*>(Cv + (tid >> 1) * STEM_CW * STEM_CP + (tid & 1) * 8) = z8;
    h8 a[7];
#pragma unroll
    for (int ky = 0; ky < 7; ++ky) a[ky] = *reinterpret_cast<const h8*>(wp + ((size_t)(r * 7 + ky) * 16 + n) * 32 + 8 * q);
    const h4 bb = *reinterpret_cast<const h4*>(bias + 4 * q);
    __syncthreads();

    const int c = 4 * n + r;
    const _Float16* bp = In + 8 * (3 * n + (6 * r + 7) / 8 + q);
#pragma unroll 3
    for (int cr = 0; cr < STEM_CR; ++cr) {
        f4 d = { 0.f, 0.f, 0.f, 0.f };
#pragma unroll
        for (int ky = 0; ky < 7; ++ky)
            d = __builtin_amdgcn_mfma_f32_16x16x32_f16(a[ky], *reinterpret_cast<const h8*>(bp + (2 * cr + ky) * STEM_PITCH), d, 0, 0, 0);
        const int gr = cv_r0 + cr;
        h4 o;
#pragma unroll
        for (int j = 0; j < 4; ++j) {
            const float f = (float)(_Float16)d[j] + (float)bb[j];
            o[j] = (gr >= 0 && gr < OHc) ? (_Float16)(f > 0.f ? f : 0.f) : (_Float16)0.f;
        }
        *reinterpret_cast<h4a4*>(Cv + ((size_t)(cr * STEM_CW + c + 1) * STEM_CP + 4 * q)) = o;
    }
    __syncthreads();

    {
        const int c8 = tid & 1, pc = (tid >> 1) & 31, pr = tid >> 6;
        if (j0 + pr < OHp) {
            h8 m = *reinterpret_cast<const h8a4*>(Cv + ((size_t)((2 * pr) * STEM_CW + 2 * pc) * STEM_CP + c8 * 8));
#pragma unroll
            for (int ky = 0; ky < 3; ++ky)
#pragma unroll
                for (int kx = 0; kx < 3; ++kx) {
                    const h8 v = *reinterpret_cast<const h8a4*>(Cv + ((size_t)((2 * pr + ky) * STEM_CW + 2 * pc + kx) * STEM_CP + c8 * 8));
#pragma unroll
                    for (int k = 0; k < 8; ++k) m[k] = v[k] > m[k] ? v[k] : m[k];
                }
            reinterpret_cast<h8*>(y)[(((size_t)img * OHp + j0 + pr) * 32 + pc) * 2 + c8] = m;
            if (w1c) *reinterpret_cast<h8*>(In + (size_t)(pr * 32 + pc) * 24 + c8 * 8) = m;
        }
    }
    if (!w1c) return;
    __syncthreads();
    if (j0 + r < OHp) {
        const bool kv = q < 2;
        const h8 aw = kv ? *reinterpret_cast<const h8*>(w1c + n * 16 + 8 * q) : z8;
        const h4 a0 = { aw[0], aw[1], aw[2], aw[3] }, a1 = { aw[4], aw[5], aw[6], aw[7] };
        const h4 b1 = *reinterpret_cast<const h4*>(b1c + 4 * q);
#pragma unroll
        for (int pt = 0; pt < 2; ++pt) {
            const h8 bv = kv ? *reinterpret_cast<const h8*>(In + (size_t)(r * 32 + pt * 16 + n) * 24 + 8 * q) : z8;
            const h4 v0 = { bv[0], bv[1], bv[2], bv[3] }, v1 = { bv[4], bv[5], bv[6], bv[7] };
            f4 d = { 0.f, 0.f, 0.f, 0.f };
            d = __builtin_amdgcn_mfma_f32_16x16x16f16(a0, v0, d, 0, 0, 0);
            d = __builtin_amdgcn_mfma_f32_16x16x16f16(a1, v1, d, 0, 0, 0);
            h4 o;
#pragma unroll
            for (int j = 0; j < 4; ++j) {
                const float f = (float)(_Float16)d[j] + (float)b1[j];
                o[j] = (_Float16)(f > 0.f ? f : 0.f);
            }
            *reinterpret_cast<h4*>(y1 + (((size_t)img * OHp + j0 + r) * 32 + pt * 16 + n) * 16 + 4 * q) = o;
        }
    }
}

#define C0_PITCH 400
#define C0_ROWS 8

template <int COUT>
__global__ __launch_bounds__(256) void k_conv0(const __half* __restrict__ x, const __half* __restrict__ wp, const __half* __restrict__ bias,
                                              __half* __restrict__ y, int H, int W, int act)
// ... 1004 lines not shown
#pragma unroll
        for (int pt = 0; pt < 2; ++pt) acc2[mt][pt] = f4{ 0.f, 0.f, 0.f, 0.f };
#pragma unroll
    for (int ks = 0; ks < KS2; ++ks) {
        h8 bv[2];
#pragma unroll
        for (int pt = 0; pt < 2; ++pt) bv[pt] = *reinterpret_cast<const h8*>(tile + (pt * 16 + n) * EP + ks * 32 + 8 * q);
#pragma unroll
        for (int mt = 0; mt < MT2; ++mt) {
            const h8 a = *reinterpret_cast<const h8*>(Ws4 + (mt * 16 + n) * EP + ks * 32 + 8 * q);
            const h4 a0 = { a[0], a[1], a[2], a[3] }, a1 = { a[4], a[5], a[6], a[7] };
#pragma unroll
            for (int pt = 0; pt < 2; ++pt) {
                const h4 b0 = { bv[pt][0], bv[pt][1], bv[pt][2], bv[pt][3] }, b1 = { bv[pt][4], bv[pt][5], bv[pt][6], bv[pt][7] };
                acc2[mt][pt] = __builtin_amdgcn_mfma_f32_16x16x16f16(a0, b0, acc2[mt][pt], 0, 0, 0);
                acc2[mt][pt] = __builtin_amdgcn_mfma_f32_16x16x16f16(a1, b1, acc2[mt][pt], 0, 0, 0);
            }
        }
    }
    __builtin_amdgcn_wave_barrier();
#pragma unroll
    for (int pt = 0; pt < 2; ++pt)
#pragma unroll
        for (int mt = 0; mt < MT2; ++mt)
            if (mt * 16 + 4 * q < N2) {
                const h4 o = { (_Float16)acc2[mt][pt][0], (_Float16)acc2[mt][pt][1], (_Float16)acc2[mt][pt][2], (_Float16)acc2[mt][pt][3] };
                *reinterpret_cast<h4*>(tile + (pt * 16 + n) * EP + mt * 16 + 4 * q) = o;
            }
    __builtin_amdgcn_wave_barrier();
#pragma unroll
    for (int it = 0; it < (32 * CG2 + 63) / 64; ++it) {
        const int i = it * 64 + lane, row = i / CG2, cg = i - row * CG2;
        if (i >= 32 * CG2) break;
        const size_t px = px0 + row;
        const h8 v = *reinterpret_cast<const h8*>(tile + row * EP + cg * 8);
        const h8 bb = *reinterpret_cast<const h8*>(Bs + 2 * C2 + cg * 8);
        h8 o;
#pragma unroll
        for (int j = 0; j < 8; ++j) {
            const float f = (float)v[j] + (float)bb[j];
            o[j] = (_Float16)(f > 0.f ? f : 0.f);
        }
        if (!pool) *reinterpret_cast<h8*>(out2 + px * N2 + cg * 8) = o;
        else *reinterpret_cast<h8*>(tile + row * EP + cg * 8) = o;
    }
    if (!pool) return;
    __syncthreads();
    {
        const int OWp = W / 2, r0 = (int)((px_wg - (size_t)img * HW) / W);
        for (int i = tid; i < 32 * CG2; i += 256) {
            const int pp = i / CG2, cg = i - pp * CG2, pr = pp / OWp, pc = pp - pr * OWp, l00 = 2 * pr * W + 2 * pc;
            const h8 a = *reinterpret_cast<const h8*>(Et + (size_t)l00 * EP + cg * 8);
            const h8 b = *reinterpret_cast<const h8*>(Et + (size_t)(l00 + 1) * EP + cg * 8);
            const h8 c = *reinterpret_cast<const h8*>(Et + (size_t)(l00 + W) * EP + cg * 8);
            const h8 d = *reinterpret_cast<const h8*>(Et + (size_t)(l00 + W + 1) * EP + cg * 8);
            h8 o;
#pragma unroll
            for (int k = 0; k < 8; ++k) o[k] = (_Float16)(((((float)a[k] + (float)b[k]) + (float)c[k]) + (float)d[k]) / 4.0f);
            const size_t op = (size_t)img * (HW / 4) + (size_t)(r0 / 2 + pr) * OWp + pc;
            *reinterpret_cast<h8*>(out2 + op * N2 + cg * 8) = o;
        }
    }
}

#define PSA_MAXT 16
__global__ __launch_bounds__(256) void k_psa_attn(const __half* __restrict__ qkv, const __half* __restrict__ pe, __half* __restrict__ out,
                                                 int N, int heads, float scale)
{
    extern __shared__ __attribute__((aligned(16))) char psa_smem[];
    _Float16* VT = reinterpret_cast<_Float16*>(psa_smem);
    const int NP = (N + 31) & ~31, VP = NP + 16, NT = NP / 16;
    const int tid = threadIdx.x, lane = tid & 63, wave = tid >> 6, q = lane >> 4, n = lane & 15;
    const int h = blockIdx.y, b = blockIdx.z, CT = heads * 128, C = heads * 64;
    const __half* base = qkv + (size_t)b * N * CT + h * 128;
    for (int i = tid; i < NP * 8; i += 256) {
        const int j = i >> 3, c8 = i & 7;
        h8 v = { 0, 0, 0, 0, 0, 0, 0, 0 };
        if (j < N) v = *reinterpret_cast<const h8*>(base + (size_t)j * CT + 64 + c8 * 8);
#pragma unroll
        for (int e = 0; e < 8; ++e) VT[(c8 * 8 + e) * VP + j] = v[e];
    }
    __syncthreads();
    const int i0 = (blockIdx.x * 4 + wave) * 16;
    if (i0 >= N) return;
    const int iq = i0 + n < N ? i0 + n : N - 1;
    const h8 z8 = { 0, 0, 0, 0, 0, 0, 0, 0 };
    const h8 bq = *reinterpret_cast<const h8*>(base + (size_t)iq * CT + 8 * q);
    f4 S[PSA_MAXT];
    float m = -INFINITY;
#pragma unroll
    for (int t = 0; t < PSA_MAXT; ++t) {
        S[t] = f4{ -INFINITY, -INFINITY, -INFINITY, -INFINITY };
        if (t < NT) {
            const int j = 16 * t + n;
            const h8 ak = j < N ? *reinterpret_cast<const h8*>(base + (size_t)j * CT + 32 + 8 * q) : z8;
            const f4 d = __builtin_amdgcn_mfma_f32_16x16x32_f16(ak, bq, f4{ 0.f, 0.f, 0.f, 0.f }, 0, 0, 0);
#pragma unroll
            for (int e = 0; e < 4; ++e) {
                S[t][e] = 16 * t + 4 * q + e < N ? d[e] * scale : -INFINITY;
                m = fmaxf(m, S[t][e]);
            }
        }
    }
    m = fmaxf(m, __shfl_xor(m, 16)); m = fmaxf(m, __shfl_xor(m, 32));
    float sum = 0.f;
#pragma unroll
    for (int t = 0; t < PSA_MAXT; ++t)
#pragma unroll
        for (int e = 0; e < 4; ++e) { S[t][e] = __expf(S[t][e] - m); sum += S[t][e]; }
    sum += __shfl_xor(sum, 16); sum += __shfl_xor(sum, 32);
    const float inv = 1.0f / sum;
    uint2 P[PSA_MAXT];
#pragma unroll
    for (int t = 0; t < PSA_MAXT; ++t) {
        const h4 p = { (_Float16)(S[t][0] * inv), (_Float16)(S[t][1] * inv), (_Float16)(S[t][2] * inv), (_Float16)(S[t][3] * inv) };
        P[t] = __builtin_bit_cast(uint2, p);
    }
    f4 acc[4];
#pragma unroll
    for (int ct = 0; ct < 4; ++ct) acc[ct] = f4{ 0.f, 0.f, 0.f, 0.f };
#pragma unroll
    for (int tp = 0; tp < PSA_MAXT / 2; ++tp) {
        if (2 * tp >= NT) break;
        const uint4 bp = { P[2 * tp].x, P[2 * tp].y, P[2 * tp + 1].x, P[2 * tp + 1].y };
#pragma unroll
        for (int ct = 0; ct < 4; ++ct) {
            const _Float16* vr = VT + (ct * 16 + n) * VP + 32 * tp + 4 * q;
            const uint2 a0 = *reinterpret_cast<const uint2*>(vr), a1 = *reinterpret_cast<const uint2*>(vr + 16);
            const uint4 av = { a0.x, a0.y, a1.x, a1.y };
            acc[ct] = __builtin_amdgcn_mfma_f32_16x16x32_f16(__builtin_bit_cast(h8, av), __builtin_bit_cast(h8, bp), acc[ct], 0, 0, 0);
        }
    }
    if (i0 + n < N) {
        const size_t o = ((size_t)b * N + i0 + n) * C + h * 64 + 4 * q;
#pragma unroll
        for (int ct = 0; ct < 4; ++ct) {
            f4 v = acc[ct];
            if (pe) {
                const h4 pv = *reinterpret_cast<const h4*>(pe + o + ct * 16);
#pragma unroll
                for (int e = 0; e < 4; ++e) v[e] = (float)(_Float16)v[e] + (float)pv[e];
            }
            const h4 r = { (_Float16)v[0], (_Float16)v[1], (_Float16)v[2], (_Float16)v[3] };
            *reinterpret_cast<h4*>(out + o + ct * 16) = r;
        }
    }
}

template <int C>
__global__ __launch_bounds__(256) void k_osnet_head(const __half* __restrict__ x, const __half* __restrict__ w, const __half* __restrict__ bias,
                                                   __half* __restrict__ out, int N, int HW, int F, const int* __restrict__ nvalid)
{
    constexpr int CR = 4, C8 = C / 8, PG = 256 / C8;
    __shared__ float part[CR][PG][C];
    __shared__ __attribute__((aligned(16))) _Float16 mean[CR][C];
    const int tid = threadIdx.x, n0 = blockIdx.x * CR;
    const int nv = nvalid ? min(*nvalid, N) : N;
    if (n0 >= nv) return;
    const int c8 = tid % C8, pg = tid / C8;
    float a[CR][8];
#pragma unroll
    for (int cr = 0; cr < CR; ++cr)
#pragma unroll
        for (int k = 0; k < 8; ++k) a[cr][k] = 0.f;
    for (int p = pg; p < HW; p += PG) {
        h8 v[CR];
#pragma unroll
        for (int cr = 0; cr < CR; ++cr)
            v[cr] = n0 + cr < nv ? *reinterpret_cast<const h8*>(x + (((size_t)(n0 + cr) * HW + p) * C + c8 * 8)) : h8{ 0, 0, 0, 0, 0, 0, 0, 0 };
#pragma unroll
        for (int cr = 0; cr < CR; ++cr)
#pragma unroll
            for (int k = 0; k < 8; ++k) a[cr][k] += (float)v[cr][k];
    }
#pragma unroll
    for (int cr = 0; cr < CR; ++cr)
#pragma unroll
        for (int k = 0; k < 8; ++k) part[cr][pg][c8 * 8 + k] = a[cr][k];
    __syncthreads();
    for (int i = tid; i < CR * C; i += 256) {
        const int cr = i / C, c = i - cr * C;
        float t = 0.f;
        for (int g = 0; g < PG; ++g) t += part[cr][g][c];
        mean[cr][c] = (_Float16)(t / (float)HW);
    }
    __syncthreads();
    for (int o = tid; o < F; o += 256) {
        float acc[CR];
#pragma unroll
        for (int cr = 0; cr < CR; ++cr) acc[cr] = 0.f;
        const h8* wr = reinterpret_cast<const h8*>(w + (size_t)o * C);
#pragma unroll 4
        for (int k8 = 0; k8 < C8; ++k8) {
            const h8 wv = wr[k8];
#pragma unroll
            for (int cr = 0; cr < CR; ++cr) {
                const h8 mv = *reinterpret_cast<const h8*>(&mean[cr][k8 * 8]);
#pragma unroll
                for (int k = 0; k < 8; ++k) acc[cr] = fmaf((float)wv[k], (float)mv[k], acc[cr]);
            }
        }
        const float b = __half2float(bias[o]);
#pragma unroll
        for (int cr = 0; cr < CR; ++cr)
            if (n0 + cr < nv) {
                const float f = (float)(_Float16)acc[cr] + b;
                out[(size_t)(n0 + cr) * F + o] = __float2half(f > 0.f ? f : 0.f);
            }
    }
}

static inline int grid_for(size_t n, int block) { size_t g = (n + block - 1) / block; return (int)(g > 4096 ? 4096 : (g ? g : 1)); }

extern "C" int ss_op_bias_act_f16(void* stream, void* x, const void* bias, const void* res, long long n_pix, int C, int act)
{
    if (!x || !bias || C < 1) return SS_ERR_INVALID;
    hipStream_t st = (hipStream_t)stream;
    if (C % 8 == 0) {
        size_t nv = (size_t)n_pix * (C / 8);
        hipLaunchKernelGGL(k_bias_act8, dim3(grid_for(nv, 256)), dim3(256), 0, st, (__half*)x, (const __half*)bias, (const __half*)res, nv, C / 8, act);
    } else {
        size_t n = (size_t)n_pix * C;
        hipLaunchKernelGGL(k_bias_act1, dim3(grid_for(n, 256)), dim3(256), 0, st, (__half*)x, (const __half*)bias, (const __half*)res, n, C, act);
    }
    return hipGetLastError() == hipSuccess ? SS_OK : SS_ERR_HIP;
}

extern "C" int ss_op_dwconv3x3_f16(void* stream, const void* x, const void* w9, const void* bias, void* y, int N, int H, int W, int C, int act)
{
    if (!x || !w9 || !bias || !y || C % 8) return SS_ERR_INVALID;
    size_t total = (size_t)N * H * W * (C / 8);
    hipLaunchKernelGGL(k_dw3x3, dim3(grid_for(total, 256)), dim3(256), 0, (hipStream_t)stream, (const __half*)x, (const __half*)w9,
                       (const __half*)bias, (__half*)y, N, H, W, C / 8, act);
    return hipGetLastError() == hipSuccess ? SS_OK : SS_ERR_HIP;
}

extern "C" int ss_op_bias_act_place_f16(void* stream, const void* x, const void* bias, const void* res, long long n_pix, int C,
                                        int act, int res_after, void* out, int out_ld, void* out2, int c0, int cn)
{
    if (!x || !bias || !out || C < 8 || C % 8 || out_ld % 8 || out_ld < C || c0 % 8 || cn % 8 || (out2 && (cn < 8 || c0 + cn > C)))
        return SS_ERR_INVALID;
    const size_t nv = (size_t)n_pix * (C / 8);
    hipLaunchKernelGGL(k_bias_act_place, dim3(grid_for(nv, 256)), dim3(256), 0, (hipStream_t)stream, (const __half*)x,
                       (const __half*)bias, (const __half*)res, nv, C / 8, act, res_after, (__half*)out, out_ld / 8,
                       (__half*)out2, c0 / 8, cn / 8);
    return hipGetLastError() == hipSuccess ? SS_OK : SS_ERR_HIP;
}

extern "C" int ss_op_v8_decode_ext_f16(void* stream, const void* const* box, const void* const* cls, const void* const* box_bias,
                                       const void* const* cls_bias, const void* const* ext, int n_ext, int ext_ld, int ext_mode,
                                       const int* H, const int* W, const int* strides, int B, int nc, int cls_ld, float* pred)
{
    if (!box || !cls || !box_bias || !cls_bias || !H || !W || !strides || !pred || B < 1 || B > 65535 || nc < 1 || cls_ld < nc) return SS_ERR_INVALID;
    if (n_ext < 0 || (n_ext && (!ext || ext_ld < n_ext || (ext_mode != 0 && ext_mode != 1) || (ext_mode == 1 && n_ext % 3)))) return SS_ERR_INVALID;
    V8Levels L;
    int A = 0;
    L.n_ext = n_ext; L.ext_ld = ext_ld; L.ext_mode = ext_mode; L.cls_ld = cls_ld;
    for (int l = 0; l < 3; ++l) {
        L.box[l] = (const __half*)box[l]; L.cls[l] = (const __half*)cls[l];
        L.box_bias[l] = (const __half*)box_bias[l]; L.cls_bias[l] = (const __half*)cls_bias[l];
        L.ext[l] = n_ext ? (const __half*)ext[l] : nullptr;
        L.H[l] = H[l]; L.W[l] = W[l]; L.stride[l] = strides[l];
        A += H[l] * W[l];
    }
    hipLaunchKernelGGL(k_v8_decode, dim3((A + 127) / 128, B), dim3(128), 0, (hipStream_t)stream, L, B, nc, A, pred);
    return hipGetLastError() == hipSuccess ? SS_OK : SS_ERR_HIP;
}

extern "C" int ss_op_v8_decode_f16(void* stream, const void* const* box, const void* const* cls, const void* const* box_bias,
                                   const void* const* cls_bias, const int* H, const int* W, const int* strides, int B, int nc,
                                   float* pred)
{
    return ss_op_v8_decode_ext_f16(stream, box, cls, box_bias, cls_bias, nullptr, 0, 0, 0, H, W, strides, B, nc, nc, pred);
}

static int launch_pw(hipStream_t st, bool conv3, const void* x, const void* w, const void* bias, const void* res, long long M, int K,
                     int N, int act, int res_after, void* out, int out_ld, void* out2, int c0, int cn, ConvGeom g)
{
    const bool vec_allowed = g_opt_pw_epilogue != 0;
    const bool vec = vec_allowed && out_ld % 8 == 0 && c0 % 8 == 0 && cn % 8 == 0 && ((uintptr_t)out % 16) == 0 &&
                     (!out2 || ((uintptr_t)out2 % 16) == 0) && (!res || ((uintptr_t)res % 16) == 0);
    const int nvb = conv3 ? 0 : nv_batch((void*)st);
    const int* nvp = (nvb > 0 && M % nvb == 0) ? nv_for((void*)st, nvb) : nullptr;
    const bool nv = nvp != nullptr;
    const PwArgs A{ (const __half*)x, (const __half*)w, (const __half*)bias, (const __half*)res, (int)M, K, N, act, res_after,
                    (__half*)out, out_ld, (__half*)out2, c0, cn, g, nvp, nv ? (int)(M / nvb) : 0 };
#define SS_PW(BN, PT, CV, VE)                                                                                           \
    hipLaunchKernelGGL((k_pw<BN, PT, CV, VE>), dim3((unsigned)((M + 64 * PT - 1) / (64 * PT)), (N + BN - 1) / BN), dim3(256), 0, st, A)
#define SS_PW2(BN, PT)                                                                                                  \
    do {                                                                                                                \
        if (conv3) { if (vec) SS_PW(BN, PT, true, true); else SS_PW(BN, PT, true, false); }                             \
        else { if (vec) SS_PW(BN, PT, false, true); else SS_PW(BN, PT, false, false); }                                 \
    } while (0)
    const bool splitk_allowed = g_opt_pw_splitk != 0;
    if (splitk_allowed && vec && conv3 && K >= 512 && M <= 4096) {
        const dim3 grid((unsigned)((M + 15) / 16), (N + ((N <= 32) ? 31 : 63)) / ((N <= 32) ? 32 : 64));
#define SS_SK(BN, CV) hipLaunchKernelGGL((k_pw_splitk<BN, CV>), grid, dim3(256), 0, st, A)
        if (N <= 32) { if (conv3) SS_SK(32, true); else SS_SK(32, false); }
        else { if (conv3) SS_SK(64, true); else SS_SK(64, false); }
#undef SS_SK
        return hipGetLastError() == hipSuccess ? SS_OK : SS_ERR_HIP;
    }
    const bool big = M >= 32768;
    if (N <= 32) { if (big) SS_PW2(32, 2); else SS_PW2(32, 1); }
    else if (N == 80) { if (big) SS_PW2(80, 2); else SS_PW2(80, 1); }
    else if (N <= 64 || !big) { if (big) SS_PW2(64, 2); else SS_PW2(64, 1); }
    else SS_PW2(128, 2);
#undef SS_PW2
#undef SS_PW
    return hipGetLastError() == hipSuccess ? SS_OK : SS_ERR_HIP;
}

extern "C" int ss_op_pointwise_f16(void* stream, const void* x, const void* w, const void* bias, const void* res, long long M,
                                   int K, int N, int act, int res_after, void* out, int out_ld, void* out2, int c0, int cn)
{
    if (!x || !w || !bias || !out || M < 1 || M > 0x7fffffffLL || K < 8 || K % 8 || N < 8 || N % 8 || out_ld % 4 || out_ld < N ||
        c0 % 4 || cn % 4 || (out2 && (cn < 4 || c0 + cn > N)))
        return SS_ERR_INVALID;
    return launch_pw((hipStream_t)stream, false, x, w, bias, res, M, K, N, act, res_after, out, out_ld, out2, c0, cn, ConvGeom{});
}

extern "C" int ss_op_conv3x3_f16(void* stream, const void* x, const void* w, const void* bias, const void* res, int B, int H, int W,
                                 int Cin, int N, int conv_stride, int act, int res_after, void* out, int out_ld, void* out2, int c0,
                                 int cn)
{
    if (!x || !w || !bias || !out || B < 1 || H < 1 || W < 1 || Cin < 8 || Cin % 8 || N < 8 || N % 8 || (conv_stride != 1 && conv_stride != 2) ||
        out_ld % 4 || out_ld < N || c0 % 4 || cn % 4 || (out2 && (cn < 4 || c0 + cn > N)))
        return SS_ERR_INVALID;
    ConvGeom g{ H, W, Cin, (H - 1) / conv_stride + 1, (W - 1) / conv_stride + 1, conv_stride };
    const long long M = (long long)B * g.OH * g.OW;
    if (M > 0x7fffffffLL) return SS_ERR_INVALID;
    return launch_pw((hipStream_t)stream, true, x, w, bias, res, M, 9 * Cin, N, act, res_after, out, out_ld, out2, c0, cn, g);
}

extern "C" int ss_op_osnet_stem_f16(void* stream, const void* x, const void* w_prep, const void* bias, void* y, int N, int H, int W,
                                    const void* w1, const void* b1, void* y1)
{
    if (!x || !w_prep || !bias || !y || N < 1 || W != STEM_W || H < 16 || H % 16 || (w1 && (!b1 || !y1))) return SS_ERR_INVALID;
    const int tiles = H / 16;
    hipLaunchKernelGGL(k_osnet_stem, dim3((unsigned)((size_t)N * tiles)), dim3(256), 0, (hipStream_t)stream, (const __half*)x,
                       (const __half*)w_prep, (const __half*)bias, (__half*)y, H, tiles, nv_for(stream, N),
                       (const __half*)w1, (const __half*)b1, (__half*)y1);
    return hipGetLastError() == hipSuccess ? SS_OK : SS_ERR_HIP;
}

extern "C" int ss_op_lightconv_f16(void* stream, const void* x, const void* w1, const void* w9, const void* bias, void* y,
                                   int N, int H, int W, int C)
{
    if (!x || !w1 || !w9 || !bias || !y || N < 1 || H < 1 || W < 8 || W % 8) return SS_ERR_INVALID;
    const size_t lds = (size_t)(LC_TH + 2) * (W + 2) * (((C + 15) / 16) * 16) * 2;
    if (lds > 65536) return SS_ERR_INVALID;
    const int bands = (H + LC_TH - 1) / LC_TH;
    hipStream_t st = (hipStream_t)stream;
    dim3 grid((unsigned)((size_t)N * bands)), block(256);
#define SS_LC(CC) hipLaunchKernelGGL(k_lightconv<CC>, grid, block, lds, st, (const __half*)x, (const __half*)w1, \
                                     (const __half*)w9, (const __half*)bias, (__half*)y, H, W, bands)
    if (C == 16) SS_LC(16);
    else if (C == 24) SS_LC(24);
    else if (C == 32) SS_LC(32);
    else return SS_ERR_INVALID;
#undef SS_LC
    return hipGetLastError() == hipSuccess ? SS_OK : SS_ERR_HIP;
}

extern "C" int ss_op_maxpool_f16(void* stream, const void* x, void* y, int N, int H, int W, int C, int k, int stride, int pad)
{
    if (!x || !y || C % 8 || k < 1 || stride < 1) return SS_ERR_INVALID;
    const int OH = (H + 2 * pad - k) / stride + 1, OW = (W + 2 * pad - k) / stride + 1;
    size_t total = (size_t)N * OH * OW * (C / 8);
    hipLaunchKernelGGL(k_maxpool, dim3(grid_for(total, 256)), dim3(256), 0, (hipStream_t)stream, (const __half*)x, (__half*)y,
                       N, H, W, C / 8, k, stride, pad, OH, OW);
    return hipGetLastError() == hipSuccess ? SS_OK : SS_ERR_HIP;
}

extern "C" int ss_op_gate_sum_f16(void* stream, const void* const* xs, int T, const void* w1, const void* b1, const void* w2,
                                  const void* b2, float* means_ws, void* out, int N, int HW, int C, int Cr)
{
    if (T < 1 || T > 4 || C % 8 || C > 256 || Cr < 1 || Cr > 16) return SS_ERR_INVALID;
    GatePtrs p;
    for (int t = 0; t < 4; ++t) p.x[t] = (const __half*)xs[t < T ? t : 0];
    hipStream_t st = (hipStream_t)stream;
    hipLaunchKernelGGL(k_gate_mean, dim3(N, T), dim3(256), 0, st, p, means_ws, N, HW, C);
    const size_t nvec = (size_t)HW * (C / 8);
    hipLaunchKernelGGL(k_gate_apply, dim3(grid_for(nvec, 256) > 64 ? 64 : grid_for(nvec, 256), N), dim3(256), 0, st, p, T, means_ws, 1, 1.0f,
                       (const __half*)w1, (const __half*)b1, (const __half*)w2, (const __half*)b2, (__half*)out, N, HW, C, Cr);
    return hipGetLastError() == hipSuccess ? SS_OK : SS_ERR_HIP;
}

static bool os_chain_form(int N, int W, int C)
{
    const bool chains = g_opt_osnet_chains != 0;
    return chains && N >= 96 && ((W == 32 && C == 16) || ((W == 16 || W == 8) && (C == 16 || C == 24 || C == 32)));
}
static int os_band_rows(int N, int H, int W, int C)
{
    if (!os_chain_form(N, W, C)) return LC_TH;
    const int target = W == 32 ? 3072 : 2048;
    const int units = W == 8 ? (N + 1) / 2 : N;
    int bands = target / (2 * units);
    if (bands < 1) bands = 1;
    if (bands > (H + 7) / 8) bands = (H + 7) / 8;
    return (H + bands - 1) / bands;
}

extern "C" int ss_op_osnet_streams_bands(int N, int H, int W, int C)
{
    if (H < 1 || N < 1) return SS_ERR_INVALID;
    const int th = os_band_rows(N, H, W, C);
    return (H + th - 1) / th;
}

extern "C" long long ss_op_dwtab_bytes(int layers, int C)
{
    if (layers < 1 || (C != 16 && C != 24 && C != 32)) return SS_ERR_INVALID;
    return (long long)layers * (C == 16 ? DwTab<16>::LAYER : C == 24 ? DwTab<24>::LAYER : DwTab<32>::LAYER);
}

extern "C" int ss_op_dwtab_f16(void* stream, const void* w9, const void* bias, int layers, int C, void* out)
{
    if (!w9 || !bias || !out || ss_op_dwtab_bytes(layers, C) < 0) return SS_ERR_INVALID;
    hipStream_t st = (hipStream_t)stream;
    if (C == 16) hipLaunchKernelGGL(k_dwtab<16>, dim3(1), dim3(256), 0, st, (const __half*)w9, (const __half*)bias, layers, (char*)out);
    else if (C == 24) hipLaunchKernelGGL(k_dwtab<24>, dim3(1), dim3(256), 0, st, (const __half*)w9, (const __half*)bias, layers, (char*)out);
    else hipLaunchKernelGGL(k_dwtab<32>, dim3(1), dim3(256), 0, st, (const __half*)w9, (const __half*)bias, layers, (char*)out);
    return hipGetLastError() == hipSuccess ? SS_OK : SS_ERR_HIP;
}

extern "C" int ss_op_osnet_streams_f16(void* stream, const void* x, const void* w1, const void* dwtab,
                                       void* const* ys, float* psum, int N, int H, int W, int C)
{
    if (!x || !w1 || !dwtab || !ys || !psum || N < 1 || H < 1 || W < 8 || W % 8) return SS_ERR_INVALID;
    const int TH = os_band_rows(N, H, W, C), bands = (H + TH - 1) / TH;
    StreamOut o;
    for (int t = 0; t < 4; ++t) { if (!ys[t]) return SS_ERR_INVALID; o.y[t] = (__half*)ys[t]; }
    hipStream_t st = (hipStream_t)stream;
    const int* nv = nv_for(stream, N);
    if (os_chain_form(N, W, C)) {
        const unsigned masks = 0x69u;
        const size_t units = W == 8 ? ((size_t)N + 1) / 2 : (size_t)N;
        dim3 grid((unsigned)((units * bands + 3) / 4), 2), block(256);
#define SS_CHN(CC, NT, PR) hipLaunchKernelGGL((k_osnet_chains<CC, NT, PR>), grid, block, 0, st, (const __half*)x, (const __half*)w1, \
                                              (const char*)dwtab, o, psum, N, H, TH, bands, masks, nv)
        if (W == 32) SS_CHN(16, 2, false);
        else if (W == 16) { if (C == 16) SS_CHN(16, 1, false); else if (C == 24) SS_CHN(24, 1, false); else SS_CHN(32, 1, false); }
        else { if (C == 16) SS_CHN(16, 1, true); else if (C == 24) SS_CHN(24, 1, true); else SS_CHN(32, 1, true); }
#undef SS_CHN
        return hipGetLastError() == hipSuccess ? SS_OK : SS_ERR_HIP;
    }
    if (C != 16 && C != 24 && C != 32) return SS_ERR_INVALID;
    const int PS = ((C + 15) / 16) * 16;
    const size_t lds = (size_t)(LC_TH + 2 * OS_TMAX) * (size_t)(2 * W + 2) * PS * 2;
    if (lds > 65536) return SS_ERR_INVALID;
    dim3 grid((unsigned)((size_t)N * bands), 4), block(256);
#define SS_OS(CC) hipLaunchKernelGGL(k_osnet_streams<CC>, grid, block, lds, st, (const __half*)x, (const __half*)w1, \
                                     (const char*)dwtab, o, psum, N, H, W, bands, nv)
    if (C == 16) SS_OS(16);
    else if (C == 24) SS_OS(24);
    else SS_OS(32);
#undef SS_OS
    return hipGetLastError() == hipSuccess ? SS_OK : SS_ERR_HIP;
}

extern "C" int ss_op_gate_apply_f16(void* stream, const void* const* xs, int T, const void* w1, const void* b1, const void* w2,
                                    const void* b2, const float* sums, int parts, float scale, void* out, int N, int HW, int C,
                                    int Cr)
{
    if (T < 1 || T > 4 || C % 8 || C > 256 || Cr < 1 || Cr > 16 || parts < 1 || !sums || !out) return SS_ERR_INVALID;
    GatePtrs p;
    for (int t = 0; t < 4; ++t) p.x[t] = (const __half*)xs[t < T ? t : 0];
    const size_t nvec = (size_t)HW * (C / 8);
    hipLaunchKernelGGL(k_gate_apply, dim3(grid_for(nvec, 256) > 64 ? 64 : grid_for(nvec, 256), N), dim3(256), 0, (hipStream_t)stream,
                       p, T, sums, parts, scale, (const __half*)w1, (const __half*)b1, (const __half*)w2, (const __half*)b2,
                       (__half*)out, N, HW, C, Cr);
    return hipGetLastError() == hipSuccess ? SS_OK : SS_ERR_HIP;
}

extern "C" int ss_op_avgpool2_f16(void* stream, const void* x, void* y, int N, int H, int W, int C)
{
    if (!x || !y || C % 8 || H < 2 || W < 2 || H % 2 || W % 2) return SS_ERR_INVALID;
    size_t total = (size_t)N * (H / 2) * (W / 2) * (C / 8);
    hipLaunchKernelGGL(k_avgpool2, dim3(grid_for(total, 256)), dim3(256), 0, (hipStream_t)stream, (const __half*)x, (__half*)y, N, H, W, C / 8);
    return hipGetLastError() == hipSuccess ? SS_OK : SS_ERR_HIP;
}

extern "C" int ss_op_osnet_tail_f16(void* stream, const void* const* ys, const float* psum, int parts, float scale, const void* gw1,
                                    const void* gb1, const void* gw2, const void* gb2, int Cr, float* gates_ws, const void* w3,
                                    const void* b3, const void* idn, int C1, const void* wd, const void* bd, void* out, const void* w4,
                                    const void* b4, void* out2, int pool, int N, int H, int W, int MID, int C2, int N2)
{
    if (!ys || !psum || !gw1 || !gb1 || !gw2 || !gb2 || !gates_ws || !w3 || !b3 || !idn || !w4 || !b4 || !out2 || parts < 1 || Cr < 1 ||
        Cr > 16 || N < 1 || H < 1 || W < 2 || (H * W) % 128 || 128 % W || (pool && ((128 / W) % 2 || W % 2)) || MID > 32 ||
        (C1 > 0 && (!wd || !bd)))
        return SS_ERR_INVALID;
    GatePtrs p;
    for (int t = 0; t < 4; ++t) { if (!ys[t]) return SS_ERR_INVALID; p.x[t] = (const __half*)ys[t]; }
    const dim3 grid((unsigned)((size_t)N * H * W / 128)), block(256);
    hipStream_t st = (hipStream_t)stream;
    const int* nv = nv_for(stream, N);
    hipLaunchKernelGGL(k_gate_vec, dim3(N), dim3(128), 0, st, psum, parts, scale, (const __half*)gw1, (const __half*)gb1,
                       (const __half*)gw2, (const __half*)gb2, Cr, MID, N, gates_ws, nv);
#define SS_TAIL(A, B, CC, DD)                                                                                                   \
    hipLaunchKernelGGL((k_osnet_tail<A, B, CC, DD>), grid, block, 0, st, p, (const float*)gates_ws, (const __half*)w3,          \
                       (const __half*)b3, (const __half*)idn, (const __half*)wd, (const __half*)bd, (__half*)out, (const __half*)w4, \
                       (const __half*)b4, (__half*)out2, pool, N, H * W, W, nv)
    if (C1 == 0) {
        if (MID == 16 && C2 == 64 && N2 == 16) SS_TAIL(16, 64, 16, 0);
        else if (MID == 16 && C2 == 64 && N2 == 64) SS_TAIL(16, 64, 64, 0);
        else if (MID == 24 && C2 == 96 && N2 == 24) SS_TAIL(24, 96, 24, 0);
        else if (MID == 24 && C2 == 96 && N2 == 96) SS_TAIL(24, 96, 96, 0);
        else if (MID == 32 && C2 == 128 && N2 == 32) SS_TAIL(32, 128, 32, 0);
        else if (MID == 32 && C2 == 128 && N2 == 128) SS_TAIL(32, 128, 128, 0);
        else return SS_ERR_INVALID;
    } else {
        if (MID == 16 && C2 == 64 && N2 == 16 && C1 == 16) SS_TAIL(16, 64, 16, 16);
        else if (MID == 24 && C2 == 96 && N2 == 24 && C1 == 64) SS_TAIL(24, 96, 24, 64);
        else if (MID == 32 && C2 == 128 && N2 == 32 && C1 == 96) SS_TAIL(32, 128, 32, 96);
        else return SS_ERR_INVALID;
    }
#undef SS_TAIL
    return hipGetLastError() == hipSuccess ? SS_OK : SS_ERR_HIP;
}

extern "C" int ss_op_conv_group_f16(void* stream, int n, const ss_conv_desc* d)
{
    if (!d || n < 1 || n > PW_GROUP_MAX) return SS_ERR_INVALID;
    const bool splitk_allowed = g_opt_pw_splitk != 0;
    const bool conv3 = d[0].ksize == 3;
    int nmax = 0, order[PW_GROUP_MAX];
    long long cost[PW_GROUP_MAX];
    PwGroup G;
    for (int i = 0; i < n; ++i) {
        const ss_conv_desc& c = d[i];
        if (!c.x || !c.w || !c.bias || !c.out || (c.ksize != 1 && c.ksize != 3) || (c.ksize == 3) != conv3 || c.B < 1 || c.H < 1 || c.W < 1 ||
            c.Cin < 8 || c.Cin % 8 || c.N < 8 || c.N % 8 || c.N > 80 || (c.stride != 1 && c.stride != 2) || (c.ksize == 1 && c.stride != 1) ||
            ((uintptr_t)c.out % 16) || ((uintptr_t)c.x % 16) || ((uintptr_t)c.w % 16))
            return SS_ERR_INVALID;
        if (c.N > nmax) nmax = c.N;
        order[i] = i;
        cost[i] = (long long)c.ksize * c.ksize * c.Cin;
    }
    for (int i = 1; i < n; ++i)
        for (int j = i; j > 0 && cost[order[j]] > cost[order[j - 1]]; --j) { const int t = order[j]; order[j] = order[j - 1]; order[j - 1] = t; }
    int wgs = 0;
    for (int s = 0; s < n; ++s) {
        const ss_conv_desc& c = d[order[s]];
        ConvGeom g{ c.H, c.W, c.Cin, (c.H - 1) / c.stride + 1, (c.W - 1) / c.stride + 1, c.stride };
        const long long M = (long long)c.B * g.OH * g.OW;
        if (M > 0x7fffffffLL) return SS_ERR_INVALID;
        const int K = c.ksize * c.ksize * c.Cin;
        G.p[s] = PwArgs{ (const __half*)c.x, (const __half*)c.w, (const __half*)c.bias, nullptr, (int)M, K, c.N, c.act, 0, (__half*)c.out,
                         c.N, nullptr, 0, 0, g, nullptr, 0 };
        G.form[s] = (splitk_allowed && conv3 && K >= 512 && M <= 4096) ? 1 : 0;
        G.start[s] = wgs;
        wgs += (int)(G.form[s] == 1 ? (M + 15) / 16 : (M + 63) / 64);
    }
    for (int s = n; s < PW_GROUP_MAX; ++s) { G.p[s] = G.p[0]; G.form[s] = 0; G.start[s] = wgs; }
    G.start[PW_GROUP_MAX] = wgs;
    G.n = n;
    hipStream_t st = (hipStream_t)stream;
    bool any_splitk = false;
    for (int s = 0; s < n; ++s) any_splitk = any_splitk || G.form[s] == 1;
#define SS_GRP(BN) do { if (conv3 && any_splitk) hipLaunchKernelGGL((k_pw_group<BN, true, true>), dim3(wgs), dim3(256), 0, st, G);            \
                        else if (conv3) hipLaunchKernelGGL((k_pw_group<BN, true, false>), dim3(wgs), dim3(256), 0, st, G);                    \
                        else hipLaunchKernelGGL((k_pw_group<BN, false, false>), dim3(wgs), dim3(256), 0, st, G); } while (0)
    if (nmax <= 32) SS_GRP(32);
    else if (nmax <= 64) SS_GRP(64);
    else SS_GRP(80);
#undef SS_GRP
    return hipGetLastError() == hipSuccess ? SS_OK : SS_ERR_HIP;
}

extern "C" int ss_op_upcat_f16(void* stream, const void* lo, const void* hi, void* out, int B, int h, int w, int C1, int C2, int lo_first)
{
    if (!lo || !hi || !out || B < 1 || h < 1 || w < 1 || C1 < 8 || C1 % 8 || C2 < 8 || C2 % 8) return SS_ERR_INVALID;
    const size_t total = (size_t)B * 4 * h * w * ((C1 + C2) / 8);
    hipLaunchKernelGGL(k_upcat, dim3(grid_for(total, 256)), dim3(256), 0, (hipStream_t)stream, (const __half*)lo, (const __half*)hi,
                       (__half*)out, B, h, w, C1 / 8, C2 / 8, lo_first);
    return hipGetLastError() == hipSuccess ? SS_OK : SS_ERR_HIP;
}

extern "C" int ss_op_osnet_head_f16(void* stream, const void* x, const void* w, const void* bias, void* out, int N, int HW, int C, int F)
{
    if (!x || !w || !bias || !out || N < 1 || HW < 1 || C != 128 || F < 1) return SS_ERR_INVALID;
    hipLaunchKernelGGL(k_osnet_head<128>, dim3((N + 3) / 4), dim3(256), 0, (hipStream_t)stream, (const __half*)x, (const __half*)w,
                       (const __half*)bias, (__half*)out, N, HW, F, nv_for(stream, N));
    return hipGetLastError() == hipSuccess ? SS_OK : SS_ERR_HIP;
}

extern "C" int ss_op_psa_attention_f16(void* stream, const void* qkv, const void* pe, void* out, int B, int N, int heads, float scale)
{
    if (!qkv || !out || B < 1 || B > 65535 || N < 1 || N > 16 * PSA_MAXT || heads < 1 || heads > 64) return SS_ERR_INVALID;
    const int NP = (N + 31) & ~31;
    hipLaunchKernelGGL(k_psa_attn, dim3((N + 63) / 64, heads, B), dim3(256), (size_t)64 * (NP + 16) * 2, (hipStream_t)stream,
                       (const __half*)qkv, (const __half*)pe, (__half*)out, N, heads, scale);
    return hipGetLastError() == hipSuccess ? SS_OK : SS_ERR_HIP;
}

extern "C" int ss_op_sppf_pools_f16(void* stream, const void* x, void* out, int B, int H, int W, int C)
{
    if (!x || !out || B < 1 || H < 1 || W < 1 || C < 8 || C % 8 || H * W > 1024) return SS_ERR_INVALID;
    hipLaunchKernelGGL(k_sppf_pools, dim3((unsigned)(B * (C / 8))), dim3(256), (size_t)2 * H * W * 16, (hipStream_t)stream,
                       (const __half*)x, (__half*)out, H, W, C / 8);
    return hipGetLastError() == hipSuccess ? SS_OK : SS_ERR_HIP;
}

extern "C" int ss_op_conv0_f16(void* stream, const void* x, const void* w_prep, const void* bias, void* y, int B, int H, int W, int Cout,
                               int act)
{
    if (!x || !w_prep || !bias || !y || B < 1 || H < 2 || W < 128 || W % 128 || (W * 3) % 8 || (Cout != 16 && Cout != 32 && Cout != 48))
        return SS_ERR_INVALID;
    const int OH = (H - 1) / 2 + 1;
    const dim3 grid(W / 128, (OH + C0_ROWS - 1) / C0_ROWS, B), block(256);
    hipStream_t st = (hipStream_t)stream;
#define SS_C0(CO) hipLaunchKernelGGL(k_conv0<CO>, grid, block, 0, st, (const __half*)x, (const __half*)w_prep, (const __half*)bias, (__half*)y, H, W, act)
    if (Cout == 16) SS_C0(16); else if (Cout == 32) SS_C0(32); else SS_C0(48);
#undef SS_C0
    return hipGetLastError() == hipSuccess ? SS_OK : SS_ERR_HIP;
}

extern "C" int ss_op_bottleneck_f16(void* stream, const void* x, const void* w1, const void* b1, const void* w2, const void* b2, int B, int H,
                                    int W, int C, int add, void* out, int out_ld, void* out2)
{
    if (!x || !w1 || !b1 || !w2 || !b2 || !out || B < 1 || H < 1 || W < 1 || (C != 16 && C != 32 && C != 64 && C != 128) || out_ld < C || out_ld % 4 ||
        ((uintptr_t)out % 8) || ((uintptr_t)x % 16) || ((uintptr_t)w1 % 16) || ((uintptr_t)w2 % 16) || (out2 && ((uintptr_t)out2 % 8)))
        return SS_ERR_INVALID;
    const long long M = (long long)B * H * W;
    const bool big = M / 128 >= 512 && C <= 64;
    BnArgs A{ (const __half*)x, (const __half*)w1, (const __half*)b1, (const __half*)w2, (const __half*)b2, (__half*)out, out_ld, (__half*)out2,
              B, H, W, add, big ? 16 : 8, 8, 0, 0 };
    A.tiles_x = (W + A.TW - 1) / A.TW; A.tiles_y = (H + A.TH - 1) / A.TH;
    const int P = C + 8;
    const size_t lds = ((size_t)(A.TH + 4) * (A.TW + 4) * P + (((size_t)(A.TH + 2) * (A.TW + 2) * P + 7) & ~(size_t)7) + 2 * (size_t)C * 72) * 2 + 128;
    const dim3 grid((unsigned)(B * A.tiles_x * A.tiles_y));
    hipStream_t st = (hipStream_t)stream;
#define SS_BN(CC, P1, P2) do { static unsigned long long attr = 0; int dv_ = 0; (void)hipGetDevice(&dv_); if (!(attr >> (dv_ & 63) & 1)) { (void)hipFuncSetAttribute((const void*)k_bneck<CC, P1, P2>, hipFuncAttributeMaxDynamicSharedMemorySize, 160 * 1024 - 512); attr |= 1ull << (dv_ & 63); }    \
                               hipLaunchKernelGGL((k_bneck<CC, P1, P2>), grid, dim3(256), lds, st, A); } while (0)
    if (big) { if (C == 16) SS_BN(16, 3, 2); else if (C == 32) SS_BN(32, 3, 2); else SS_BN(64, 3, 2); }
    else { if (C == 16) SS_BN(16, 2, 1); else if (C == 32) SS_BN(32, 2, 1); else if (C == 64) SS_BN(64, 2, 1); else SS_BN(128, 2, 1); }
#undef SS_BN
    return hipGetLastError() == hipSuccess ? SS_OK : SS_ERR_HIP;
}

extern "C" int ss_op_head_f16(void* stream, const void* x, const void* const* w1, const void* const* b1, const void* const* w2,
                              const void* const* b2, const void* const* w3, const void* const* b3, void* const* out, const int* nout,
                              int B, int H, int W, int Cin, int tile16)
{
    if (!x || !w1 || !b1 || !w2 || !b2 || !w3 || !b3 || !out || !nout || B < 1 || H < 1 || W < 1 || (Cin != 64 && Cin != 128 && Cin != 256) ||
        ((uintptr_t)x % 16))
        return SS_ERR_INVALID;
    HeadArgs A;
    A.x = (const __half*)x;
    for (int b = 0; b < 2; ++b) {
        const int cm = b ? 80 : 64;
        if (!w1[b] || !b1[b] || !w2[b] || !b2[b] || !w3[b] || !b3[b] || !out[b] || nout[b] < 8 || nout[b] % 8 || nout[b] > cm ||
            ((uintptr_t)w1[b] % 16) || ((uintptr_t)w2[b] % 16) || ((uintptr_t)w3[b] % 16) || ((uintptr_t)out[b] % 8))
            return SS_ERR_INVALID;
        A.w1[b] = (const __half*)w1[b]; A.b1[b] = (const __half*)b1[b]; A.w2[b] = (const __half*)w2[b]; A.b2[b] = (const __half*)b2[b];
        A.w3[b] = (const __half*)w3[b]; A.b3[b] = (const __half*)b3[b]; A.out[b] = (__half*)out[b]; A.nout[b] = nout[b];
    }
    const bool big = tile16 != 0 && Cin == 64;
    A.B = B; A.H = H; A.W = W; A.TW = big ? 16 : 8; A.TH = 8;
    A.tiles_x = (W + A.TW - 1) / A.TW; A.tiles_y = (H + A.TH - 1) / A.TH;
    const size_t xs = ((size_t)(A.TH + 4) * (A.TW + 4) * (Cin + 8) + 7) & ~(size_t)7, ts = ((size_t)(A.TH + 2) * (A.TW + 2) * 88 + 7) & ~(size_t)7;
    const size_t lds = (xs + ts + 2 * 80 * 72) * 2 + 128;
    if (lds > 160 * 1024 - 512) return SS_ERR_INVALID;
    const dim3 grid((unsigned)(B * A.tiles_x * A.tiles_y), 2);
    hipStream_t st = (hipStream_t)stream;
#define SS_HD(CC, P1, P2) do { static unsigned long long attr = 0; int dv_ = 0; (void)hipGetDevice(&dv_); if (!(attr >> (dv_ & 63) & 1)) { (void)hipFuncSetAttribute((const void*)k_head<CC, P1, P2>, hipFuncAttributeMaxDynamicSharedMemorySize, 160 * 1024 - 512); attr |= 1ull << (dv_ & 63); }    \
                               hipLaunchKernelGGL((k_head<CC, P1, P2>), grid, dim3(256), lds, st, A); } while (0)
    if (big) SS_HD(64, 3, 2);
    else if (Cin == 64) SS_HD(64, 2, 1);
    else if (Cin == 128) SS_HD(128, 2, 1);
    else SS_HD(256, 2, 1);
#undef SS_HD
    return hipGetLastError() == hipSuccess ? SS_OK : SS_ERR_HIP;
}

extern "C" int ss_op_set_valid_images(void* stream, const int* d_n, int batch)
{
    NvEntry* slot = nullptr;
    for (NvEntry& e : g_nv) if (e.n && e.stream == stream) slot = &e;
    if (!d_n) { if (slot) *slot = NvEntry{}; return SS_OK; }
    if (batch < 1) return SS_ERR_INVALID;
    if (!slot) for (NvEntry& e : g_nv) if (!e.n) { slot = &e; break; }
    if (!slot) return SS_ERR_CAPACITY;
    *slot = NvEntry{ stream, d_n, batch };
    return SS_OK;
}

extern "C" int ss_op_set_option(const char* name, int value)
{
    if (!name) return SS_ERR_INVALID;
    const std::string n(name);
    if (n == "pw_epilogue") g_opt_pw_epilogue = value;
    else if (n == "pw_splitk") g_opt_pw_splitk = value;
    else if (n == "osnet_chains") g_opt_osnet_chains = value;
    else return SS_ERR_INVALID;
    return SS_OK;
}
```

Measured before the change: 8592.

## Add LDS-resident weight paths for small-K convs, bottlenecks, and vectorized front kernels

Adds several new paths. A letterbox kernel stages source rows in LDS and writes fp16 HWC output in 8-pixel vector stores. A direct u8 crop variant skips the LUT and reuses neighbouring pixel fetches. The change also adds pointwise and 3x3 conv kernels that keep the whole weight matrix resident in LDS, with A blocks preloaded into registers, and a bottleneck variant that stages both conv weights in LDS once per block instead of streaming them per k-chunk. All are gated by a new small_k_resident option that is on by default; they aim to cut repeated global weight loads and scalar byte traffic, at the cost of higher LDS and register pressure.

```diff
diff --git a/strongsort_yolo_amd/csrc/ss_front.hip b/strongsort_yolo_amd/csrc/ss_front.hip
--- a/strongsort_yolo_amd/csrc/ss_front.hip
+++ b/strongsort_yolo_amd/csrc/ss_front.hip
@@ -62,6 +62,108 @@
     }
 }
 
+#define LB_LDS_BYTES 30720
+__global__ __launch_bounds__(256) void k_letterbox_hwc8(const uint8_t* __restrict__ src, long long src_batch_stride,
+                                                        int H, int W, int stride, __half* __restrict__ dst, int out_h,
+                                                        int out_w, int new_h, int new_w, int pad_top, int pad_left,
+                                                        float padv)
+{
+    __shared__ __attribute__((aligned(16))) uint32_t Ls[LB_LDS_BYTES / 4 + 2];
+    __shared__ __half lut[256];
+    __shared__ int srow[32];
+    const int tid = threadIdx.x, xb = blockIdx.x * 128, yb = blockIdx.y * 16;
+    src += (size_t)blockIdx.z * src_batch_stride;
+    dst += (size_t)blockIdx.z * 3 * ((size_t)out_h * out_w);
+    const float sx = (float)W / (float)new_w, sy = (float)H / (float)new_h;
+    lut[tid] = ss_cvt<__half>((float)tid / 255.0f);
+    if (tid < 32) {
+        const int y = yb + (tid >> 1), ry = y - pad_top;
+        int r = -1;
+        if (y < out_h && ry >= 0 && ry < new_h) { int y0, y1; float fy; ss_axis(ry, sy, H, y0, y1, fy); r = (tid & 1) ? y1 : y0; }
+        srow[tid] = r;
+    }
+    const int rxa = max(xb - pad_left, 0), rxb = min(xb + 127 - pad_left, new_w - 1);
+    int ca0 = 0, ca1 = 0, cb0 = 0, cb1 = 0; float fa, fb;
+    if (rxa <= rxb) { ss_axis(rxa, sx, W, ca0, ca1, fa); ss_axis(rxb, sx, W, cb0, cb1, fb); }
+    const size_t rowb = (size_t)ca0 * 3;
+    const int mis = (int)(rowb & 3), ndw = (mis + (cb1 - ca0 + 1) * 3 + 3) >> 2, pitch = ndw + 1;
+    const bool staged = (stride & 3) == 0 && ((uintptr_t)src & 3) == 0 && (size_t)32 * pitch * 4 <= LB_LDS_BYTES;
+    __syncthreads();
+    if (staged && rxa <= rxb) {
+        const size_t end = (size_t)H * stride;
+        const int tot = 32 * ndw;
+        for (int i0 = tid; i0 < tot; i0 += 256 * 8) {
+            uint32_t v[8];
+            int la[8];
+#pragma unroll
+            for (int u = 0; u < 8; ++u) {
+                const int i = i0 + 256 * u;
+                v[u] = 0; la[u] = -1;
+                if (i < tot) {
+                    const int rr = i / ndw, dw = i - rr * ndw, sr = srow[rr];
+                    if (sr >= 0) {
+                        const size_t off = (size_t)sr * stride + (rowb - mis) + (size_t)dw * 4;
+                        la[u] = rr * pitch + dw;
+                        if (off + 4 <= end) v[u] = *reinterpret_cast<const uint32_t*>(src + off);
+                        else { for (int k = 0; k < 4 && off + k < end; ++k) v[u] |= (uint32_t)src[off + k] << (8 * k); }
+                    }
+                }
+            }
+#pragma unroll
+            for (int u = 0; u < 8; ++u) if (la[u] >= 0) Ls[la[u]] = v[u];
+        }
+    }
+    __syncthreads();
+    const int row = tid >> 4, y = yb + row, xg = xb + (tid & 15) * 8;
+    if (y >= out_h || xg >= out_w) return;
+    const int ry = y - pad_top;
+    const __half padh = ss_cvt<__half>(padv);
+    __attribute__((aligned(16))) __half o[24];
+#pragma unroll
+    for (int i = 0; i < 24; ++i) o[i] = padh;
+    if (ry >= 0 && ry < new_h) {
+        int y0, y1; float fy;
+        ss_axis(ry, sy, H, y0, y1, fy);
+        const uint32_t* l0 = Ls + (2 * row) * pitch;
+        const uint32_t* l1 = l0 + pitch;
+        const uint8_t* r0 = src + (size_t)y0 * stride;
+        const uint8_t* r1 = src + (size_t)y1 * stride;
+        auto px = [&](const uint32_t* lrow, int ob) -> uint32_t {
+            const int dw = ob >> 2;
+            const uint64_t two = ((uint64_t)lrow[dw + 1] << 32) | lrow[dw];
+            return (uint32_t)(two >> (8 * (ob & 3)));
+        };
+        auto gpx = [&](const uint8_t* grow, int xx) -> uint32_t {
+            return (uint32_t)grow[xx * 3] | ((uint32_t)grow[xx * 3 + 1] << 8) | ((uint32_t)grow[xx * 3 + 2] << 16);
+        };
+#pragma unroll
+        for (int p = 0; p < 8; ++p) {
+            const int rx = xg + p - pad_left;
+            if (rx < 0 || rx >= new_w) continue;
+            int x0, x1; float fx;
+            ss_axis(rx, sx, W, x0, x1, fx);
+            uint32_t v00, v01, v10, v11;
+            if (staged) {
+                const int ob0 = mis + 3 * (x0 - ca0), ob1 = mis + 3 * (x1 - ca0);
+                v00 = px(l0, ob0); v01 = px(l0, ob1); v10 = px(l1, ob0); v11 = px(l1, ob1);
+            } else { v00 = gpx(r0, x0); v01 = gpx(r0, x1); v10 = gpx(r1, x0); v11 = gpx(r1, x1); }
+#pragma unroll
+            for (int c = 0; c < 3; ++c) {
+                const int sh = 8 * (2 - c);
+                const float p00 = (float)((v00 >> sh) & 255u), p01 = (float)((v01 >> sh) & 255u), p10 = (float)((v10 >> sh) & 255u),
+                            p11 = (float)((v11 >> sh) & 255u);
+                o[p * 3 + c] = lut[(int)ss_bilerp_u8(p00, p01, p10, p11, fx, fy)];
+            }
+        }
+    }
+    uint4* out = reinterpret_cast<uint4*>(dst + ((size_t)y * out_w + xg) * 3);
+    const uint4* ov = reinterpret_cast<const uint4*>(o);
+#pragma unroll
+    for (int v = 0; v < 3; ++v) out[v] = ov[v];
+}
+
+int ss_front_vec = 6;
+
 void ss_launch_letterbox(const uint8_t* src, int batch, long long src_batch_stride, int h, int w, int stride, void* dst,
                          int flags, int out_h, int out_w, int new_h, int new_w, int pad_top, int pad_left,
                          int pad_value, hipStream_t st)
@@ -69,6 +171,11 @@
     if (batch <= 0) return;
     dim3 grid((out_w + 255) / 256, out_h, batch), block(256);
     float padv = (float)pad_value / 255.0f;
+    if ((flags & 3) == 3 && (ss_front_vec & 2) && out_w % 8 == 0 && ((uintptr_t)dst % 16) == 0) {
+        hipLaunchKernelGGL(k_letterbox_hwc8, dim3((out_w + 127) / 128, (out_h + 15) / 16, batch), block, 0, st, src, src_batch_stride, h, w,
+                           stride, (__half*)dst, out_h, out_w, new_h, new_w, pad_top, pad_left, padv);
+        return;
+    }
 #define SS_LB(T, L) hipLaunchKernelGGL((k_letterbox<T, L>), grid, block, 0, st, src, src_batch_stride, h, w, stride, \
                                        (T*)dst, out_h, out_w, new_h, new_w, pad_top, pad_left, padv)
     switch (flags & 3) {
@@ -122,15 +229,15 @@
 #define CROP_LDS_BYTES 30720
 #define CROP_RPT 4
 
-template <typename T>
-__global__ __launch_bounds__(256) void k_crop_hwc8(const uint8_t* __restrict__ src, long long src_batch_stride, int H, int W,
+template <typename T, bool DIRECT = false>
+__global__ __launch_bounds__(256) __attribute__((amdgpu_waves_per_eu(DIRECT ? 3 : 1))) void k_crop_hwc8(const uint8_t* __restrict__ src, long long src_batch_stride, int H, int W,
                                                    int stride, const float* __restrict__ dets, int det_stride,
                                                    long long dets_batch_stride, int n, const int* __restrict__ d_count,
                                                    T* __restrict__ dst, const int* __restrict__ d_off)
 {
     extern __shared__ __attribute__((aligned(16))) unsigned char crop_smem[];
     T* lut = reinterpret_cast<T*>(crop_smem);
-    uint32_t* Ls = reinterpret_cast<uint32_t*>(crop_smem + 768 * sizeof(T));
+    uint32_t* Ls = reinterpret_cast<uint32_t*>(crop_smem + (DIRECT ? 0 : 768 * sizeof(T)));
     const int out_w = 128, out_h = 256;
     const int img = blockIdx.z / n, d = blockIdx.z - img * n;
     const int cnt = d_count ? d_count[img] : n;
@@ -146,7 +253,7 @@
     if (cw < 1) cw = 1; if (ch < 1) ch = 1;
     const float sx = (float)cw / (float)out_w, sy = (float)ch / (float)out_h;
     const float mean[3] = { 0.485f, 0.456f, 0.406f }, sd[3] = { 0.229f, 0.224f, 0.225f };
-    for (int i = tid; i < 768; i += 256) {
+    for (int i = tid; i < 768 && !DIRECT; i += 256) {
         const int c = i >> 8;
         const float q = (float)(i & 255) / 255.0f;
         if constexpr (ss_is_u8<T>::value) lut[i] = (uint8_t)(i & 255);
@@ -202,12 +309,17 @@
         ss_axis(xg + p, sx, cw, xx0, xx1, hfx[p]);
         hob0[p] = mis + 3 * xx0; hob1[p] = mis + 3 * xx1;
     }
+    bool chained = DIRECT;
+#pragma unroll
+    for (int p = 1; p < 8; ++p) chained = chained && (hob0[p] == hob0[p - 1] || hob0[p] == hob1[p - 1]);
+    const bool share = DIRECT && __all(chained);
 #pragma unroll 1
     for (int rr = 0; rr < CROP_RPT; ++rr) {
     const int y = yb + rr * 16 + (tid >> 4);
     int yy0, yy1; float fy;
     ss_axis(y, sy, ch, yy0, yy1, fy);
     __attribute__((aligned(16))) T o[24];
+    uint32_t ow[6] = { 0, 0, 0, 0, 0, 0 };
     if (staged) {
         int row0 = ra0;
         if (mode == 1) {
@@ -225,31 +337,43 @@
             const uint64_t two = ((uint64_t)row[dw + 1] << 32) | row[dw];
             return (uint32_t)(two >> (8 * (ob & 3)));
         };
+        uint32_t q00 = 0, q01 = 0, q10 = 0, q11 = 0;
 #pragma unroll
         for (int p = 0; p < 8; ++p) {
             const float fx = hfx[p];
-            const uint32_t v00 = px(l0, hob0[p]), v01 = px(l0, hob1[p]), v10 = px(l1, hob0[p]), v11 = px(l1, hob1[p]);
+            uint32_t v00, v10;
+            int ob0 = hob0[p], ob1 = hob1[p];
+            if (share && p > 0) { const bool same = hob0[p] == hob0[p - 1]; v00 = same ? q00 : q01; v10 = same ? q10 : q11; }
+            else { v00 = px(l0, ob0); v10 = px(l1, ob0); }
+            const uint32_t v01 = px(l0, ob1), v11 = px(l1, ob1);
+            q00 = v00; q01 = v01; q10 = v10; q11 = v11;
 #pragma unroll
             for (int c = 0; c < 3; ++c) {
                 const int sh = 8 * (2 - c);
                 const float p00 = (float)((v00 >> sh) & 255u), p01 = (float)((v01 >> sh) & 255u), p10 = (float)((v10 >> sh) & 255u),
                             p11 = (float)((v11 >> sh) & 255u);
-                o[p * 3 + c] = lut[c * 256 + (int)ss_bilerp_u8(p00, p01, p10, p11, fx, fy)];
+                const int qv = (int)ss_bilerp_u8(p00, p01, p10, p11, fx, fy);
+                if constexpr (DIRECT) ow[(p * 3 + c) >> 2] |= (uint32_t)qv << (8 * ((p * 3 + c) & 3));
+                else o[p * 3 + c] = lut[c * 256 + qv];
             }
         }
     } else {
         const uint8_t* r0 = src + (size_t)(y1 + yy0) * stride + rowb;
         const uint8_t* r1 = src + (size_t)(y1 + yy1) * stride + rowb;
         T* od = dst + (slot * out_h * out_w + (size_t)y * out_w + xg) * 3;
+        int np = 8;
+        if constexpr (DIRECT) asm volatile("" : "+s"(np));
 #pragma unroll 1
-        for (int p = 0; p < 8; ++p) {
+        for (int p = 0; p < np; ++p) {
             int xx0, xx1; float fx;
             ss_axis(xg + p, sx, cw, xx0, xx1, fx);
 #pragma unroll
             for (int c = 0; c < 3; ++c) {
                 const int sc = 2 - c;
                 const float p00 = r0[xx0 * 3 + sc], p01 = r0[xx1 * 3 + sc], p10 = r1[xx0 * 3 + sc], p11 = r1[xx1 * 3 + sc];
-                od[p * 3 + c] = lut[c * 256 + (int)ss_bilerp_u8(p00, p01, p10, p11, fx, fy)];
+                const int qv = (int)ss_bilerp_u8(p00, p01, p10, p11, fx, fy);
+                if constexpr (DIRECT) od[p * 3 + c] = (T)qv;
+                else od[p * 3 + c] = lut[c * 256 + qv];
             }
         }
         continue;
@@ -258,7 +382,7 @@
         uint2* out = reinterpret_cast<uint2*>(dst + (slot * out_h * out_w + (size_t)y * out_w + xg) * 3);
         const uint2* ov = reinterpret_cast<const uint2*>(o);
 #pragma unroll
-        for (int v = 0; v < 3; ++v) out[v] = ov[v];
+        for (int v = 0; v < 3; ++v) out[v] = DIRECT ? make_uint2(ow[2 * v], ow[2 * v + 1]) : ov[v];
     } else {
         constexpr int NV = 24 * sizeof(T) / 16;
         uint4* out = reinterpret_cast<uint4*>(dst + (slot * out_h * out_w + (size_t)y * out_w + xg) * 3);
@@ -333,6 +457,7 @@
     if (n <= 0 || batch <= 0) return;
     if (flags & 2) {
         dim3 grid(1, 16 / CROP_RPT, n * batch), block(256);
+        if ((flags & 4) && (ss_front_vec & 4)) { hipLaunchKernelGGL((k_crop_hwc8<uint8_t, true>), grid, block, CROP_LDS_BYTES + 8, st, frame, frame_batch_stride, h, w, stride, dets, det_stride, dets_batch_stride, n, d_count, (uint8_t*)out, d_off); return; }
         if (flags & 4) { hipLaunchKernelGGL(k_crop_hwc8<uint8_t>, grid, block, 768 + CROP_LDS_BYTES + 8, st, frame, frame_batch_stride, h, w, stride, dets, det_stride, dets_batch_stride, n, d_count, (uint8_t*)out, d_off); return; }
         if (flags & 1) hipLaunchKernelGGL(k_crop_hwc8<__half>, grid, block, 768 * sizeof(__half) + CROP_LDS_BYTES + 8, st, frame, frame_batch_stride, h, w, stride, dets, det_stride, dets_batch_stride, n, d_count, (__half*)out, d_off);
         else           hipLaunchKernelGGL(k_crop_hwc8<float>, grid, block, 768 * sizeof(float) + CROP_LDS_BYTES + 8, st, frame, frame_batch_stride, h, w, stride, dets, det_stride, dets_batch_stride, n, d_count, (float*)out, d_off);
diff --git a/strongsort_yolo_amd/csrc/ss_ops.hip b/strongsort_yolo_amd/csrc/ss_ops.hip
--- a/strongsort_yolo_amd/csrc/ss_ops.hip
+++ b/strongsort_yolo_amd/csrc/ss_ops.hip
@@ -19,6 +19,10 @@
 }
 
 static int g_opt_pw_epilogue = 1, g_opt_pw_splitk = 1, g_opt_osnet_chains = 1;
+enum { SK_LETTERBOX = 2, SK_CROP_U8 = 4, SK_PW3_32 = 8, SK_PW3_64 = 16, SK_PW1_64 = 32, SK_BNECK16 = 64, SK_BNECK32 = 128 };
+#define SK_DEFAULT (SK_LETTERBOX | SK_CROP_U8 | SK_PW3_32 | SK_PW3_64 | SK_PW1_64 | SK_BNECK16 | SK_BNECK32)
+static int g_opt_small_k = SK_DEFAULT;
+extern int ss_front_vec;
 
 typedef _Float16 h8 __attribute__((ext_vector_type(8)));
 typedef _Float16 h4 __attribute__((ext_vector_type(4)));
@@ -210,9 +214,19 @@
 template <int BN, int PT, bool VEC_EPI>
 constexpr int pw_lds_halfs() { return BN * 72 + (VEC_EPI ? 4 * PT * 16 * (BN + 8) : 0); }
 
-template <int BN, int PT, bool CONV3, bool VEC_EPI>
+#define PW_RES_BYTES 36864
+__host__ __device__ inline int pw_res_kp(int K) { return K + 8 + (((K >> 3) & 1) ? 8 : 0); }
+template <int BN> __host__ __device__ inline bool pw_res_overlay(int K) { return BN * pw_res_kp(K) > 8192; }
+template <int BN, int PT> __host__ __device__ inline int pw_res_lds_halfs(int K)
+{
+    const int wh = BN * pw_res_kp(K), th = 4 * PT * 16 * (BN + 8);
+    return pw_res_overlay<BN>(K) ? (wh > th ? wh : th) : wh + th;
+}
+
+template <int BN, int PT, bool CONV3, bool VEC_EPI, bool RES = false, int NB = 0>
 __device__ __forceinline__ void pw_body(const PwArgs& A, const int bx, const int by, _Float16* __restrict__ pw_lds)
 {
+    static_assert(!RES || VEC_EPI, "the resident form has the vector epilogue only");
     const __half* __restrict__ x = A.x; const __half* __restrict__ w = A.w; const __half* __restrict__ bias = A.bias;
     const __half* __restrict__ res = A.res; __half* __restrict__ out = A.out; __half* __restrict__ out2 = A.out2;
     const int K = A.K, N = A.N, act = A.act, res_after = A.res_after, out_ld = A.out_ld, c0 = A.c0, cn = A.cn;
@@ -271,23 +285,109 @@
             }
     };
     h8 wr[WV], wn[WV], b[KC / 32][PT], bn[KC / 32][PT];
-    load_w(0, wr);
-    load_b(0, b);
+    const int KP = RES ? pw_res_kp(K) : PITCH;
+    h8 bias0 = z8;
+    if (RES) { const int oc = n0 + (lane % (BN / 8)) * 8; if (oc < N) bias0 = *reinterpret_cast<const h8*>(bias + oc); }
+    if constexpr (RES && NB > 0) {
+        constexpr int RV = (BN * NB * 4 + 255) / 256;
+        const int K8 = K >> 3, tot = BN * K8;
+        constexpr int NB1 = NB > 6 ? 5 : NB;
+        h8 ball[NB][PT], t[RV];
+        auto load_blocks = [&](const int kb0, const int kb1) {
+#pragma unroll
+        for (int kb = 0; kb < NB; ++kb)
+#pragma unroll
+            for (int pt = 0; pt < PT; ++pt) {
+                if (kb < kb0 || kb >= kb1) continue;
+                const size_t px = px0 + pt * 16 + n;
+                const int k = kb * 32 + 8 * q;
+                if (!CONV3) {
+                    ball[kb][pt] = (px < (size_t)M && k < K) ? *reinterpret_cast<const h8*>(x + px * K + k) : z8;
+                } else {
+                    const int tap = k / g.Cin, c = k - tap * g.Cin, dy = tap / 3, dx = tap - dy * 3;
+                    const int iy = iy0[pt] + dy, ix = ix0[pt] + dx;
+                    const bool ok = px < (size_t)M && k < K && iy >= 0 && iy < g.H && ix >= 0 && ix < g.W;
+                    ball[kb][pt] = ok ? *reinterpret_cast<const h8*>(x + (ibase[pt] + (size_t)iy * g.W + ix) * g.Cin + c) : z8;
+                }
+            }
+        };
+        load_blocks(0, NB1);
+#pragma unroll
+        for (int j = 0; j < RV; ++j) {
+            const int i = tid + j * 256, r = i / K8, c8 = i - r * K8, oc = n0 + r;
+            t[j] = (i < tot && oc < N) ? *reinterpret_cast<const h8*>(w + (size_t)oc * K + c8 * 8) : z8;
+        }
+#pragma unroll
+        for (int j = 0; j < RV; ++j) {
+            const int i = tid + j * 256, r = i / K8, c8 = i - r * K8;
+            if (i < tot) *reinterpret_cast<h8*>(Ws + r * KP + c8 * 8) = t[j];
+        }
+        load_blocks(NB1, NB);
+        __syncthreads();
+#pragma unroll
+        for (int kb = 0; kb < NB; ++kb) {
+            const int k = kb * 32 + 8 * q;
+#pragma unroll
+            for (int mt = 0; mt < MT; ++mt) {
+                h8 a = *reinterpret_cast<const h8*>(Ws + (mt * 16 + n) * KP + (k < K ? k : 0));
+                if (k >= K) a = z8;
+                const h4 a0 = { a[0], a[1], a[2], a[3] }, a1 = { a[4], a[5], a[6], a[7] };
+#pragma unroll
+                for (int pt = 0; pt < PT; ++pt) {
+                    const h8 bv = ball[kb][pt];
+                    if (CONV3) {
+                        acc[mt][pt] = __builtin_amdgcn_mfma_f32_16x16x32_f16(a, bv, acc[mt][pt], 0, 0, 0);
+                    } else {
+                        const h4 b0 = { bv[0], bv[1], bv[2], bv[3] }, b1 = { bv[4], bv[5], bv[6], bv[7] };
+                        acc[mt][pt] = __builtin_amdgcn_mfma_f32_16x16x16f16(a0, b0, acc[mt][pt], 0, 0, 0);
+                        acc[mt][pt] = __builtin_amdgcn_mfma_f32_16x16x16f16(a1, b1, acc[mt][pt], 0, 0, 0);
+                    }
+                }
+            }
+        }
+    } else {
+    if (RES) {
+        constexpr int RV = PW_RES_BYTES / 16 / 256;
+        const int K8 = K >> 3, tot = BN * K8;
+        h8 t[RV];
+        load_b(0, b);
+#pragma unroll
+        for (int j = 0; j < RV; ++j) {
+            const int i = tid + j * 256, r = i / K8, c8 = i - r * K8, oc = n0 + r;
+            t[j] = (i < tot && oc < N) ? *reinterpret_cast<const h8*>(w + (size_t)oc * K + c8 * 8) : z8;
+        }
+#pragma unroll
+        for (int j = 0; j < RV; ++j) {
+            const int i = tid + j * 256, r = i / K8, c8 = i - r * K8;
+            if (i < tot) *reinterpret_cast<h8*>(Ws + r * KP + c8 * 8) = t[j];
+        }
+        __syncthreads();
+    } else {
+        load_w(0, wr);
+        load_b(0, b);
+    }
     for (int kc = 0; kc < K; kc += KC) {
-        __syncthreads();
-#pragma unroll
-        for (int j = 0; j < WV; ++j) {
-            const int i = tid + j * 256, r = i / (KC / 8), c8 = i - r * (KC / 8);
-            if (i < BN * (KC / 8)) *reinterpret_cast<h8*>(Ws + r * PITCH + c8 * 8) = wr[j];
-        }
-        if (kc + KC < K) { load_w(kc + KC, wn); load_b(kc + KC, bn); }
-        __syncthreads();
+        if (!RES) {
+            __syncthreads();
+#pragma unroll
+            for (int j = 0; j < WV; ++j) {
+                const int i = tid + j * 256, r = i / (KC / 8), c8 = i - r * (KC / 8);
+                if (i < BN * (KC / 8)) *reinterpret_cast<h8*>(Ws + r * PITCH + c8 * 8) = wr[j];
+            }
+        }
+        if (kc + KC < K) { if (!RES) load_w(kc + KC, wn); load_b(kc + KC, bn); }
+        if (!RES) __syncthreads();
 #pragma unroll
         for (int ks = 0; ks < KC / 32; ++ks) {
             if (kc + ks * 32 >= K) break;
 #pragma unroll
             for (int mt = 0; mt < MT; ++mt) {
-                const h8 a = *reinterpret_cast<const h8*>(Ws + (mt * 16 + n) * PITCH + ks * 32 + 8 * q);
+                h8 a;
+                if (RES) {
+                    const int k = kc + ks * 32 + 8 * q;
+                    a = *reinterpret_cast<const h8*>(Ws + (mt * 16 + n) * KP + (k < K ? k : 0));
+                    if (k >= K) a = z8;
+                } else a = *reinterpret_cast<const h8*>(Ws + (mt * 16 + n) * PITCH + ks * 32 + 8 * q);
                 const h4 a0 = { a[0], a[1], a[2], a[3] }, a1 = { a[4], a[5], a[6], a[7] };
 #pragma unroll
                 for (int pt = 0; pt < PT; ++pt) {
@@ -304,17 +404,20 @@
         }
         if (kc + KC < K) {
 #pragma unroll
-            for (int j = 0; j < WV; ++j) wr[j] = wn[j];
+            for (int j = 0; j < WV; ++j) if (!RES) wr[j] = wn[j];
 #pragma unroll
             for (int ks = 0; ks < KC / 32; ++ks)
 #pragma unroll
                 for (int pt = 0; pt < PT; ++pt) b[ks][pt] = bn[ks][pt];
         }
+    }
     }
 
     if (VEC_EPI) {
         constexpr int EP = BN + 8;
-        _Float16* tile = pw_lds + BN * PITCH + wave * (PT * 16 * EP);
+        const bool overlay = RES && pw_res_overlay<BN>(K);
+        if (overlay) __syncthreads();
+        _Float16* tile = pw_lds + (overlay ? 0 : BN * KP) + wave * (PT * 16 * EP);
 #pragma unroll
         for (int pt = 0; pt < PT; ++pt)
 #pragma unroll
@@ -331,7 +434,7 @@
             const int oc = n0 + cg * 8;
             if (i >= PT * 16 * CG || px >= (size_t)M || oc >= N) continue;
             const h8 v = *reinterpret_cast<const h8*>(tile + row * EP + cg * 8);
-            const h8 bb = *reinterpret_cast<const h8*>(bias + oc);
+            const h8 bb = RES ? bias0 : *reinterpret_cast<const h8*>(bias + oc);
             h8 r = z8;
             if (res) r = *reinterpret_cast<const h8*>(res + px * N + oc);
             h8 o;
@@ -386,6 +489,13 @@
 {
     __shared__ __attribute__((aligned(16))) _Float16 pw_lds[pw_lds_halfs<BN, PT, VEC_EPI>()];
     pw_body<BN, PT, CONV3, VEC_EPI>(A, blockIdx.x, blockIdx.y, pw_lds);
+}
+
+template <int BN, int PT, bool CONV3, int NB>
+__global__ __launch_bounds__(256) __attribute__((amdgpu_waves_per_eu(pw_waves<BN, PT, CONV3>()))) void k_pw_res(PwArgs A)
+{
+    extern __shared__ __attribute__((aligned(16))) _Float16 pw_res_lds[];
+    pw_body<BN, PT, CONV3, true, true, NB>(A, blockIdx.x, blockIdx.y, pw_res_lds);
 }
 
 template <int BN, bool CONV3>
@@ -574,26 +684,102 @@
     }
 }
 
-template <int C, int PT1, int PT2>
-__global__ __launch_bounds__(256) __attribute__((amdgpu_waves_per_eu(!SS_TAIL_BUMP ? 1 : C == 16 ? 6 : 1))) void k_bneck(BnArgs A)
-{
-    extern __shared__ __attribute__((aligned(16))) char bn_smem[];
+template <int CI, int CO, int PT>
+__device__ __forceinline__ void bn_conv_res(const _Float16* __restrict__ In, const int (&pbase)[PT], const int* __restrict__ tapoff,
+                                            const _Float16* __restrict__ Ws, f4 (&acc)[CO / 16][PT], const int tid)
+{
+    constexpr int C = CI, MT = CO / 16, K = 9 * CI, KP = K + 8 + (((K >> 3) & 1) ? 8 : 0);
+    const int lane = tid & 63, q = lane >> 4, n = lane & 15;
+    const h8 z8 = { 0, 0, 0, 0, 0, 0, 0, 0 };
+    auto load_ab = [&](int k0, h8 (&a)[2][MT], h8 (&b)[2][PT]) {
+#pragma unroll
+        for (int ks = 0; ks < 2; ++ks) {
+            const int kk = k0 + ks * 32 + 8 * q, tap = kk / C, c = kk % C;
+            const bool kv = kk < K;
+            const int boff = kv ? tapoff[tap] + c : 0;
+#pragma unroll
+            for (int pt = 0; pt < PT; ++pt) {
+                b[ks][pt] = *reinterpret_cast<const h8*>(In + pbase[pt] + boff);
+                if (!kv) b[ks][pt] = z8;
+            }
+#pragma unroll
+            for (int mt = 0; mt < MT; ++mt) {
+                a[ks][mt] = *reinterpret_cast<const h8*>(Ws + (mt * 16 + n) * KP + (kv ? kk : 0));
+                if (!kv) a[ks][mt] = z8;
+            }
+        }
+    };
+    h8 a[2][MT], b[2][PT], an[2][MT], bn[2][PT];
+    load_ab(0, a, b);
+#pragma unroll
+    for (int k0 = 0; k0 < K; k0 += 64) {
+        if (k0 + 64 < K) load_ab(k0 + 64, an, bn);
+#pragma unroll
+        for (int ks = 0; ks < 2; ++ks) {
+            if (k0 + ks * 32 >= K) break;
+#pragma unroll
+            for (int mt = 0; mt < MT; ++mt)
+#pragma unroll
+                for (int pt = 0; pt < PT; ++pt)
+                    acc[mt][pt] = __builtin_amdgcn_mfma_f32_16x16x32_f16(a[ks][mt], b[ks][pt], acc[mt][pt], 0, 0, 0);
+        }
+        if (k0 + 64 < K) {
+#pragma unroll
+            for (int ks = 0; ks < 2; ++ks) {
+#pragma unroll
+                for (int mt = 0; mt < MT; ++mt) a[ks][mt] = an[ks][mt];
+#pragma unroll
+                for (int pt = 0; pt < PT; ++pt) b[ks][pt] = bn[ks][pt];
+            }
+        }
+    }
+}
+
+template <int C> constexpr int bn_res_kp() { return 9 * C + 8 + ((((9 * C) >> 3) & 1) ? 8 : 0); }
+template <int C, int PT1, int PT2, bool RES>
+__device__ __forceinline__ void bneck_body(const BnArgs& A, char* bn_smem)
+{
     constexpr int MT = C / 16, P = C + 8, WP = 72;
+    constexpr int KR = bn_res_kp<C>(), RV = (C * 9 * C / 8 + 255) / 256;
     const int tid = threadIdx.x, lane = tid & 63, wave = tid >> 6, q = lane >> 4, n = lane & 15;
     const int TW = A.TW, TH = A.TH, XW = TW + 4, XH = TH + 4, RW = TW + 2, RH = TH + 2;
     _Float16* Xs = reinterpret_cast<_Float16*>(bn_smem);
     _Float16* Ts = Xs + XH * XW * P;
     _Float16* Ws = Ts + ((RH * RW * P + 7) & ~7);
-    int* tap1 = reinterpret_cast<int*>(Ws + 2 * C * WP);
+    int* tap1 = reinterpret_cast<int*>(Ws + (RES ? ((C * KR + 7) & ~7) : 2 * C * WP));
     int* tap2 = tap1 + 16;
     const int tpi = A.tiles_x * A.tiles_y;
     const int img = blockIdx.x / tpi, trm = blockIdx.x - img * tpi, tyi = trm / A.tiles_x, txi = trm - tyi * A.tiles_x;
     const int oy0 = tyi * TH, ox0 = txi * TW, H = A.H, W = A.W;
     const h8 z8 = { 0, 0, 0, 0, 0, 0, 0, 0 };
     if (tid < 9) { const int ky = tid / 3, kx = tid - ky * 3; tap1[tid] = (ky * XW + kx) * P; tap2[tid] = (ky * RW + kx) * P; }
+    h8 wv1[RV], wv2[RV];
+    if (RES) {
+#pragma unroll
+        for (int j = 0; j < RV; ++j) {
+            const int i = tid + j * 256;
+            wv1[j] = i < C * 9 * C / 8 ? *reinterpret_cast<const h8*>(A.w1 + (size_t)i * 8) : z8;
+        }
+    }
     const __half* xi = A.x + (size_t)img * H * W * C;
     constexpr int VPC = C / 8;
     const int rowv = XW * VPC;
+    if constexpr (RES) {
+        constexpr int NV = (12 * 20 * VPC + 255) / 256;
+        h8 tmp[NV];
+#pragma unroll
+        for (int u = 0; u < NV; ++u) {
+            const int i = tid + 256 * u, r = i / rowv, rem = i - r * rowv, c = rem / VPC, v = rem % VPC;
+            const int iy = oy0 - 2 + r, ix = ox0 - 2 + c;
+            const bool ok = r < XH && iy >= 0 && iy < H && ix >= 0 && ix < W;
+            tmp[u] = ok ? *reinterpret_cast<const h8*>(xi + ((size_t)iy * W + ix) * C + v * 8) : z8;
+        }
+#pragma unroll
+        for (int u = 0; u < NV; ++u) {
+            const int i = tid + 256 * u, r = i / rowv, rem = i - r * rowv, c = rem / VPC, v = rem % VPC;
+            if (r < XH) *reinterpret_cast<h8*>(Xs + (r * XW + c) * P + v * 8) = tmp[u];
+        }
+    } else
     for (int r = wave; r < XH; r += 4) {
         const int iy = oy0 - 2 + r;
         const bool rok = iy >= 0 && iy < H;
@@ -613,6 +799,22 @@
                 if (i < rowv) *reinterpret_cast<h8*>(dst + c * P + v * 8) = tmp[u];
             }
         }
+    }
+    auto store_w = [&](const h8 (&wv)[RV]) {
+#pragma unroll
+        for (int j = 0; j < RV; ++j) {
+            const int i = tid + j * 256, r = i / (9 * C / 8), c8 = i - r * (9 * C / 8);
+            if (i < C * 9 * C / 8) *reinterpret_cast<h8*>(Ws + r * KR + c8 * 8) = wv[j];
+        }
+    };
+    if (RES) {
+        store_w(wv1);
+#pragma unroll
+        for (int j = 0; j < RV; ++j) {
+            const int i = tid + j * 256;
+            wv2[j] = i < C * 9 * C / 8 ? *reinterpret_cast<const h8*>(A.w2 + (size_t)i * 8) : z8;
+        }
+        __syncthreads();
     }
     {
         int pb[PT1], tpix[PT1];
@@ -633,7 +835,8 @@
         for (int mt = 0; mt < MT; ++mt)
 #pragma unroll
             for (int pt = 0; pt < PT1; ++pt) acc[mt][pt] = f4{ 0.f, 0.f, 0.f, 0.f };
-        bn_conv<C, C, PT1>(Xs, pb, tap1, A.w1, Ws, acc, tid);
+        if constexpr (RES) bn_conv_res<C, C, PT1>(Xs, pb, tap1, Ws, acc, tid);
+        else bn_conv<C, C, PT1>(Xs, pb, tap1, A.w1, Ws, acc, tid);
 #pragma unroll
         for (int mt = 0; mt < MT; ++mt) {
             const h4 bb = *reinterpret_cast<const h4*>(A.b1 + mt * 16 + 4 * q);
@@ -652,6 +855,7 @@
         }
     }
     __syncthreads();
+    if (RES) { store_w(wv2); __syncthreads(); }
     {
         int pb[PT2], opix[PT2], xoff[PT2];
 #pragma unroll
@@ -669,7 +873,8 @@
         for (int mt = 0; mt < MT; ++mt)
 #pragma unroll
             for (int pt = 0; pt < PT2; ++pt) acc[mt][pt] = f4{ 0.f, 0.f, 0.f, 0.f };
-        bn_conv<C, C, PT2>(Ts, pb, tap2, A.w2, Ws, acc, tid);
+        if constexpr (RES) bn_conv_res<C, C, PT2>(Ts, pb, tap2, Ws, acc, tid);
+        else bn_conv<C, C, PT2>(Ts, pb, tap2, A.w2, Ws, acc, tid);
 #pragma unroll
         for (int mt = 0; mt < MT; ++mt) {
             const h4 bb = *reinterpret_cast<const h4*>(A.b2 + mt * 16 + 4 * q);
@@ -690,6 +895,20 @@
             }
         }
     }
+}
+
+template <int C, int PT1, int PT2>
+__global__ __launch_bounds__(256) __attribute__((amdgpu_waves_per_eu(!SS_TAIL_BUMP ? 1 : C == 16 ? 6 : 1))) void k_bneck(BnArgs A)
+{
+    extern __shared__ __attribute__((aligned(16))) char bn_smem[];
+    bneck_body<C, PT1, PT2, false>(A, bn_smem);
+}
+
+template <int C, int PT1, int PT2>
+__global__ __launch_bounds__(256) __attribute__((amdgpu_waves_per_eu(!SS_TAIL_BUMP ? 1 : C == 16 ? 5 : 1))) void k_bneck_res(BnArgs A)
+{
+    extern __shared__ __attribute__((aligned(16))) char bn_smem[];
+    bneck_body<C, PT1, PT2, true>(A, bn_smem);
 }
 
 struct HeadArgs {
@@ -2300,6 +2519,17 @@
         return hipGetLastError() == hipSuccess ? SS_OK : SS_ERR_HIP;
     }
     const bool big = M >= 32768;
+    if (vec && big && !nv && K > 64 && N <= 64 && (N <= 32 ? 32 : 64) * K * 2 <= PW_RES_BYTES &&
+        (g_opt_small_k & (!conv3 ? (N <= 32 ? 0 : SK_PW1_64) : N <= 32 ? SK_PW3_32 : SK_PW3_64))) {
+#define SS_PWR(BN, CV, NB) hipLaunchKernelGGL((k_pw_res<BN, 2, CV, NB>), dim3((unsigned)((M + 127) / 128), (N + BN - 1) / BN), dim3(256),      \
+                                          ((size_t)pw_res_lds_halfs<BN, 2>(K) * 2), st, A)
+        const int nb = (K + 31) / 32;
+        if (N <= 32) { if (nb == 5) SS_PWR(32, true, 5); else SS_PWR(32, true, 0); }
+        else if (conv3) { if (nb == 9) SS_PWR(64, true, 9); else SS_PWR(64, true, 0); }
+        else { if (nb == 4) SS_PWR(64, false, 4); else if (nb == 6) SS_PWR(64, false, 6); else SS_PWR(64, false, 0); }
+#undef SS_PWR
+        return hipGetLastError() == hipSuccess ? SS_OK : SS_ERR_HIP;
+    }
     if (N <= 32) { if (big) SS_PW2(32, 2); else SS_PW2(32, 1); }
     else if (N == 80) { if (big) SS_PW2(80, 2); else SS_PW2(80, 1); }
     else if (N <= 64 || !big) { if (big) SS_PW2(64, 2); else SS_PW2(64, 1); }
@@ -2631,6 +2861,13 @@
     const size_t lds = ((size_t)(A.TH + 4) * (A.TW + 4) * P + (((size_t)(A.TH + 2) * (A.TW + 2) * P + 7) & ~(size_t)7) + 2 * (size_t)C * 72) * 2 + 128;
     const dim3 grid((unsigned)(B * A.tiles_x * A.tiles_y));
     hipStream_t st = (hipStream_t)stream;
+    if (big && C <= 32 && (g_opt_small_k & (C == 16 ? SK_BNECK16 : SK_BNECK32))) {
+        const size_t wh = C == 16 ? 16 * bn_res_kp<16>() : 32 * bn_res_kp<32>();
+        const size_t ldr = ((size_t)(A.TH + 4) * (A.TW + 4) * P + (((size_t)(A.TH + 2) * (A.TW + 2) * P + 7) & ~(size_t)7) + ((wh + 7) & ~(size_t)7)) * 2 + 128;
+        if (C == 16) hipLaunchKernelGGL((k_bneck_res<16, 3, 2>), grid, dim3(256), ldr, st, A);
+        else hipLaunchKernelGGL((k_bneck_res<32, 3, 2>), grid, dim3(256), ldr, st, A);
+        return hipGetLastError() == hipSuccess ? SS_OK : SS_ERR_HIP;
+    }
 #define SS_BN(CC, P1, P2) do { static unsigned long long attr = 0; int dv_ = 0; (void)hipGetDevice(&dv_); if (!(attr >> (dv_ & 63) & 1)) { (void)hipFuncSetAttribute((const void*)k_bneck<CC, P1, P2>, hipFuncAttributeMaxDynamicSharedMemorySize, 160 * 1024 - 512); attr |= 1ull << (dv_ & 63); }    \
                                hipLaunchKernelGGL((k_bneck<CC, P1, P2>), grid, dim3(256), lds, st, A); } while (0)
     if (big) { if (C == 16) SS_BN(16, 3, 2); else if (C == 32) SS_BN(32, 3, 2); else SS_BN(64, 3, 2); }
@@ -2693,6 +2930,7 @@
     if (n == "pw_epilogue") g_opt_pw_epilogue = value;
     else if (n == "pw_splitk") g_opt_pw_splitk = value;
     else if (n == "osnet_chains") g_opt_osnet_chains = value;
+    else if (n == "small_k_resident") { g_opt_small_k = value == 1 ? SK_DEFAULT : value < 0 ? 0 : value; ss_front_vec = g_opt_small_k & (SK_LETTERBOX | SK_CROP_U8); }
     else return SS_ERR_INVALID;
     return SS_OK;
 }
```

After: 8684, median of 2. No clear change (+1.1%).
